# W298/Surtr

Hardware: AMD Instinct MI355X
Metric: fragments/sec (higher is better)
Workload: dtype f32

## Files before the change

surtr_amd/csrc/small_clip.h:

```cpp
#pragma once
#include "clip_core.h"

#define SC_V 192u
#define SC_H 640u
#define SC_FALLBACK 101

namespace surtr {

struct ScSolid
{
    float pos[3 * SC_V];
    uint32_t vw[SC_V];
    uint32_t re[SC_H];
};

struct ScLds
{
    ScSolid buf[2];
    int8_t c[SC_V];
    uint16_t km[SC_V];
    uint16_t mp[SC_V];
    uint16_t noff[SC_V];
    uint16_t succ[SC_V], pred[SC_V];
    uint32_t nv[2], flag;
#ifdef SURTR_STAMP
    unsigned long long tph[8];
#endif
};

__device__ inline int small_clip(const SolidIn in, const uint32_t F, const Shared& sh, ScLds& L, uint32_t* which, uint32_t* stop = nullptr)
{
    const uint32_t lane = lane_id();
    const uint32_t V = in.nv;
#ifdef SURTR_STAMP
    unsigned long long sc_t0 = __builtin_readcyclecounter();
    if (lane == 0) for (int q = 0; q < 8; ++q) L.tph[q] = 0;
#define SC_STAMP(i) do { if (lane == 0) { const unsigned long long t1 = __builtin_readcyclecounter(); L.tph[i] += t1 - sc_t0; sc_t0 = t1; } } while (0)
#else
#define SC_STAMP(i) do { } while (0)
#endif
    if (stop != nullptr) *stop = 0xFFFFFFFFu;
    if (V == 0 || V > SC_V) return SC_FALLBACK;
    const uint32_t hbase = in.loff[0], H = in.loff[V - 1u] + in.llen[V - 1u] - hbase;
    if (H > SC_H) return SC_FALLBACK;
    bool odd = false;
    for (uint32_t v = lane; v < V; v += SURTR_LANES)
    {
        ScSolid& S = L.buf[0];
        S.pos[3 * v] = in.pos[3 * v]; S.pos[3 * v + 1] = in.pos[3 * v + 1]; S.pos[3 * v + 2] = in.pos[3 * v + 2];
        const uint32_t lo = in.loff[v] - hbase, deg = in.llen[v];
        if (deg > 15u || deg < 3u) odd = true;
        const uint32_t dl = deg > 15u ? 15u : deg;
        S.vw[v] = lo | (dl << 16);
        const int32_t* r = in.nbr + in.loff[v];
        for (uint32_t j = 0; j < dl && lo + j < SC_H; ++j)
        {
            if ((uint32_t)r[j] >= V) odd = true;
            S.re[lo + j] = (uint32_t)r[j] & 0xFFFFu;
            for (uint32_t jj = 0; jj < j; ++jj) if (r[jj] == r[j]) odd = true;
        }
    }
    if (__ballot(odd) != 0ull) return SC_FALLBACK;
    __syncthreads();
    for (uint32_t v = lane; v < V; v += SURTR_LANES)
    {
        ScSolid& S = L.buf[0];
        const uint32_t w = S.vw[v], lo = w & 0xFFFFu, deg = w >> 16;
        for (uint32_t j = 0; j < deg; ++j)
        {
            const uint32_t e = S.re[lo + j] & 0xFFFFu;
            const uint32_t we = S.vw[e], elo = we & 0xFFFFu, edeg = we >> 16;
            uint32_t q = 0;
            while (q < edeg && (S.re[elo + q] & 0xFFFFu) != v) ++q;
            if (q >= edeg) odd = true;
            S.re[lo + j] = e | (q << 16);
        }
    }
    if (__ballot(odd) != 0ull) return SC_FALLBACK;
    __syncthreads();
    SC_STAMP(0);
#define SC_GIVE_UP do { if (stop != nullptr) { *stop = k; *which = cur; if (lane == 0) L.nv[cur] = nv; __syncthreads(); } return SC_FALLBACK; } while (0)
    uint32_t cur = 0, nv = V;
    for (uint32_t k = 0; k < F && nv != 0u; ++k)
    {
        const float4 pl = sh.planes[k];
        ScSolid& S = L.buf[cur]; ScSolid& N = L.buf[cur ^ 1u];
        bool zero = false, cut = false, keep = false;
        for (uint32_t v = lane; v < nv; v += SURTR_LANES)
        {
            const int c = side_of(plane_dist(pl, S.pos[3 * v], S.pos[3 * v + 1], S.pos[3 * v + 2]));
            L.c[v] = (int8_t)c;
            zero = zero || c == 0; cut = cut || c < 0; keep = keep || c > 0;
        }
        const bool anyCut = __ballot(cut) != 0ull;
        if (__ballot(keep) == 0ull) { if (!anyCut) SC_GIVE_UP; nv = 0; break; }
        if (!anyCut) continue;
        if (__ballot(zero) != 0ull) SC_GIVE_UP;
        __syncthreads();
        SC_STAMP(1);
        uint32_t carryM = 0, carryK = 0, carryH = 0;
        for (uint32_t v0 = 0; v0 < nv; v0 += SURTR_LANES)
        {
            const uint32_t v = v0 + lane;
            uint32_t mask = 0, isKept = 0, deg = 0;
            if (v < nv)
            {
                const uint32_t w = S.vw[v], lo = w & 0xFFFFu;
                deg = w >> 16;
                if (L.c[v] > 0) isKept = 1u;
                else
                    for (uint32_t j = 0; j < deg; ++j) if (L.c[S.re[lo + j] & 0xFFFFu] > 0) mask |= 1u << j;
            }
            const uint32_t cnt = (uint32_t)__builtin_popcount(mask);
            const uint2 inc = wave_incl_scan2(make_uint2(cnt | (isKept << 16), isKept ? deg : 0u));
            if (v < nv)
            {
                L.km[v] = (uint16_t)mask;
                L.mp[v] = isKept ? (uint16_t)(carryK + (inc.x >> 16) - 1u) : (uint16_t)(0x8000u | (carryM + (inc.x & 0xFFFFu) - cnt));
                L.noff[v] = (uint16_t)(carryH + inc.y - (isKept ? deg : 0u));
            }
            const uint32_t tx = lane_bcast(inc.x, SURTR_LANES - 1u), ty = lane_bcast(inc.y, SURTR_LANES - 1u);
            carryM += tx & 0xFFFFu; carryK += tx >> 16; carryH += ty;
        }
        const uint32_t M = carryM, nKeep = carryK, HK = carryH;
        if (nKeep + M > SC_V || HK + 3u * M > SC_H) SC_GIVE_UP;
        if (nKeep + M < 4u) { nv = 0; break; }
        for (uint32_t t = lane; t < M; t += SURTR_LANES) L.pred[t] = 0xFFFFu;
        __syncthreads();
        SC_STAMP(2);
        bool bad = false;
        for (uint32_t v = lane; v < nv; v += SURTR_LANES)
        {
            uint32_t mask = L.c[v] < 0 ? L.km[v] : 0u;
            if (!mask) continue;
            uint32_t t = L.mp[v] & 0x7FFFu;
            const uint32_t wv = S.vw[v];
            for (; mask; mask &= mask - 1u, ++t)
            {
                uint32_t cv = v, w = wv, slot = (uint32_t)__builtin_ctz(mask), steps = 0, end = 0xFFFFu;
                while (steps++ <= nv)
                {
                    const uint32_t len = w >> 16;
                    const uint32_t p = slot == 0u ? len - 1u : slot - 1u;
                    const uint32_t rw = S.re[(w & 0xFFFFu) + p];
                    const uint32_t e = rw & 0xFFFFu;
                    if (L.c[e] > 0) { end = (L.mp[cv] & 0x7FFFu) + (uint32_t)__builtin_popcount(L.km[cv] & ((1u << p) - 1u)); break; }
                    cv = e; slot = rw >> 16; w = S.vw[e];
                }
                if (end == 0xFFFFu || end == t) { bad = true; continue; }
                L.succ[t] = (uint16_t)end;
                L.pred[end] = (uint16_t)t;
            }
        }
        if (__ballot(bad) != 0ull) SC_GIVE_UP;
        __syncthreads();
        SC_STAMP(3);
        for (uint32_t t = lane; t < M; t += SURTR_LANES) if (L.pred[t] == 0xFFFFu || L.pred[L.succ[t]] != t || L.pred[t] == L.succ[t]) bad = true;
        if (__ballot(bad) != 0ull) SC_GIVE_UP;
        SC_STAMP(4);
        for (uint32_t v = lane; v < nv; v += SURTR_LANES)
        {
            const uint32_t w = S.vw[v], lo0 = w & 0xFFFFu, deg = w >> 16;
            if (L.c[v] > 0)
            {
                const uint32_t id = L.mp[v], lo = L.noff[v];
                N.pos[3 * id] = S.pos[3 * v]; N.pos[3 * id + 1] = S.pos[3 * v + 1]; N.pos[3 * id + 2] = S.pos[3 * v + 2];
                N.vw[id] = lo | (deg << 16);
                for (uint32_t j = 0; j < deg; ++j)
                {
                    const uint32_t rw = S.re[lo0 + j], e = rw & 0xFFFFu, q = rw >> 16;
                    const uint32_t m = L.mp[e], kme = L.km[e];
                    N.re[lo + j] = (m & 0x8000u) ? (nKeep + (m & 0x7FFFu) + (uint32_t)__builtin_popcount(kme & ((1u << q) - 1u))) | (2u << 16)
                                                 : m | (q << 16);
                }
            }
            else
            {
                const float ax = S.pos[3 * v], ay = S.pos[3 * v + 1], az = S.pos[3 * v + 2];
                const float sa = plane_dist(pl, ax, ay, az);
                uint32_t t = L.mp[v] & 0x7FFFu;
                for (uint32_t mask = L.km[v]; mask; mask &= mask - 1u, ++t)
                {
                    const uint32_t rw = S.re[lo0 + (uint32_t)__builtin_ctz(mask)], u = rw & 0xFFFFu;
                    const float bx = S.pos[3 * u], by = S.pos[3 * u + 1], bz = S.pos[3 * u + 2];
                    const float sb = plane_dist(pl, bx, by, bz);
                    const float inv = 1.f / (sb - sa);
                    const uint32_t id = nKeep + t, lo = HK + 3u * t;
                    N.pos[3 * id] = (ax * sb - bx * sa) * inv;
                    N.pos[3 * id + 1] = (ay * sb - by * sa) * inv;
                    N.pos[3 * id + 2] = (az * sb - bz * sa) * inv;
                    N.vw[id] = lo | (3u << 16);
                    N.re[lo] = (nKeep + L.pred[t]) | (1u << 16); N.re[lo + 1] = (nKeep + L.succ[t]) | (0u << 16);
                    N.re[lo + 2] = (uint32_t)L.mp[u] | (rw & 0xFFFF0000u);
                }
            }
        }
        nv = nKeep + M;
        cur ^= 1u;
        __syncthreads();
        SC_STAMP(5);
#ifdef SURTR_STAMP
        if (lane == 0) L.tph[6] += 1;
#endif
    }
#undef SC_GIVE_UP
    SC_STAMP(1);
    *which = cur;
    if (lane == 0) L.nv[cur] = nv;
    __syncthreads();
    return 0;
}

__device__ inline SolidIn sc_stage(const ScSolid& S, uint32_t nv, float* pos, uint32_t* loff, uint32_t* llen, uint32_t* ring)
{
    for (uint32_t v = lane_id(); v < nv; v += SURTR_LANES)
    {
        pos[3 * v] = S.pos[3 * v]; pos[3 * v + 1] = S.pos[3 * v + 1]; pos[3 * v + 2] = S.pos[3 * v + 2];
        const uint32_t w = S.vw[v], lo = w & 0xFFFFu, len = w >> 16;
        loff[v] = lo; llen[v] = len;
        for (uint32_t q = 0; q < len; ++q) ring[lo + q] = S.re[lo + q] & 0xFFFFu;
    }
    __threadfence_block();
    __syncthreads();
    return SolidIn{pos, loff, llen, (const int32_t*)ring, nv, nullptr, nullptr, nullptr, nullptr, nullptr};
}

__device__ inline int sc_park(const ScSolid& S, uint32_t nv, Shared& sh, uint32_t* cursors, float* apos, uint32_t* aloff, uint32_t* allen, int32_t* anbr,
                              uint32_t capV, uint32_t capH, uint32_t& voff, uint32_t& n, uint32_t& hoff, uint32_t& nh)
{
    const uint32_t wl = S.vw[nv - 1u];
    const uint32_t H = (wl & 0xFFFFu) + (wl >> 16);
    __syncthreads();
    if (threadIdx.x == 0) { sh.misc[0] = atomicAdd(&cursors[CUR_V], nv); sh.misc[1] = atomicAdd(&cursors[CUR_H], H); }
    __syncthreads();
    voff = sh.misc[0]; hoff = sh.misc[1];
    __syncthreads();
    if ((uint64_t)voff + nv > capV || (uint64_t)hoff + H > capH) return SURTR_E_CAPACITY;
    for (uint32_t v = lane_id(); v < nv; v += SURTR_LANES)
    {
        const size_t id = (size_t)voff + v;
        apos[3 * id] = S.pos[3 * v]; apos[3 * id + 1] = S.pos[3 * v + 1]; apos[3 * id + 2] = S.pos[3 * v + 2];
        const uint32_t w = S.vw[v];
        const uint32_t lo = hoff + (w & 0xFFFFu), len = w >> 16;
        aloff[id] = lo; allen[id] = len;
        const uint32_t* r = S.re + (w & 0xFFFFu);
        for (uint32_t q = 0; q < len; ++q) anbr[lo + q] = (int32_t)(r[q] & 0xFFFFu);
    }
    n = nv; nh = H;
    __syncthreads();
    return 0;
}

}
```

surtr_amd/csrc/surtr_ctx.h:

```cpp
#pragma once
#include <algorithm>
#include <chrono>
#include <cstdint>
#include <cstdlib>
#include <string>
#include <vector>

#include "../../include/surtr_hip.h"
#include "clip_core.h"

using namespace surtr;

struct PairRec
{
    uint32_t cv_off, cv_n, ch_off, ch_n;
    uint32_t mv_off, mv_n, mh_off, mh_n;
    uint32_t ni, isl_off;
    uint32_t status;
    uint32_t img_fmt, img_off, img_n, img_h, img_pc;
    uint32_t cv_bad;
};

enum { IMG_NONE = 0,
       IMG_NARROW = 1,
       IMG_WIDE = 2,
       IMG_EMPTY = 3,
       IMG_REC = 4 };

struct ImgLayout { uint32_t hist, zhist, nzero, mask, loff, llen, comp, ring, pos, total; };
__host__ __device__ static inline ImgLayout img_layout(uint32_t F, uint32_t nbV, uint32_t n, uint32_t hsum, uint32_t posCap = 0)
{
    auto up = [](uint32_t b) { return (b + 15u) & ~15u; };
    ImgLayout L;
    L.hist = 0; L.zhist = up(4u * F); L.nzero = L.zhist + up(4u * F); L.mask = L.nzero + up(4u * F); L.loff = L.mask + up(8u * nbV);
    L.llen = L.loff + up(2u * n); L.comp = L.llen + up(n); L.ring = L.comp + up(n); L.pos = L.ring + up(2u * hsum);
    L.total = L.pos + up(12u * (n > posCap ? n : posCap));
    return L;
}

struct ImgArena { char* base; uint32_t cap16; };

struct PrepPool { char* base; size_t per_wg; uint32_t VMAX; };
static size_t prep_bytes_per_wg(uint32_t VMAX)
{
    auto r = [](size_t b) { return (b + 255) & ~(size_t)255; };
    return 2 * r((size_t)VMAX * 4) + r((size_t)(VMAX / SURTR_SB + 2) * 4) + 2 * r((size_t)(VMAX / SURTR_LANES + 2) * 8) +
           2 * r((size_t)VMAX + 64) +
           2 * r((size_t)VMAX * 4) +
           r((size_t)VMAX * 2 + 64);
}

struct FragRec
{
    int32_t cell, piece, island;
    uint32_t mv_off, mv_n, mh_off, mh_n;
    uint32_t cv_off, cv_n, ch_off, ch_n;
    uint32_t idx_off, idx_n;
    uint32_t o_mv, o_mh, o_cv, o_ch, o_idx;
};

struct Arena
{
    float* pos; uint32_t* loff; uint32_t* llen; int32_t* nbr; uint32_t* idx;
    uint2* isl;
    uint32_t capV, capH, capI, capIsl;
    uint32_t* cursors;
};

enum : uint32_t
{
    CUR_V = 0,
    CUR_H = 1,
    CUR_I = 2,
    CUR_ISL = 3,
    CUR_Q_CLIP = 4,
    CUR_STATUS = 5,
    CUR_Q_REFIT = 6,
    CUR_Q_FACES = 7,
    CUR_Q_CONVEX = 8,
    CUR_Q_PREP = 9,
    CUR_IMG = 10,
    CUR_Q_BIG = 11,
    CUR_Q_HALF = 12,
    CUR_Q_RETRY = 13,
    CUR_FLAGGED_FRAGS = 14,
    CUR_FLAGGED_PAIRS = 15,
    CUR_CLS_CLIP = 16,
    CUR_CLS_FRAG = 32,
    CUR_CLS_PREP = 48,
    CUR_CLS_HALF = 64,
    CUR_RETRY_N = CUR_CLS_HALF,
    CUR_CVX_RESUMED = 78,
    CUR_REFIT_RESUMED = 79,
    CUR_CVX_TOOK = 80,
    CUR_REFIT_TOOK = 82,
    CUR_BIG_QUOTA = 84,
    CUR_FACES2_N = 85,
    CUR_Q_FACES2 = 86,
    CUR_REC_TOOK = 88,
    CUR_REC_HANDED = 89,
    CUR_LIT_TOO_LARGE = 90,
    CUR_REC_IMAGES = 91,
    CUR_SORTED_SEL = 92,
    CUR_REC_SPENT = 93,
    CUR_CATCH_CLIPPED = 94,
    CUR_UNREFITTED = 95,
    CUR_WC_WHY = 96,
    CUR_STATS_WORDS = 128,
    CUR_HO_PUSHED = 146,
    CUR_HO_STARTED = 147,
    CUR_HO_SIGNED_OFF = 148,
    CUR_HO_POLL_SLOT = 149,
    CUR_Q_CATCH = 150,
    CUR_Q_SWEEP = 151,
    CUR_HO_WORDS = 6,
    CUR_COUNT = 256
};
static_assert(CUR_V == 0 && CUR_H == 1 && CUR_I == 2 && CUR_ISL == 3 && CUR_STATUS == 5 && CUR_CLS_CLIP == 16 && CUR_CLS_FRAG == 32 &&
              CUR_CLS_PREP == 48 && CUR_CLS_HALF == 64 && CUR_REC_TOOK == 88 && CUR_REC_HANDED == 89 && CUR_LIT_TOO_LARGE == 90 &&
              CUR_UNREFITTED == 95 && CUR_WC_WHY == 96, "include/surtr_hip.h publishes these slots of surtr_queue_stats by number");
static_assert(CUR_STATS_WORDS <= CUR_COUNT && CUR_Q_SWEEP + 1 == CUR_HO_PUSHED + CUR_HO_WORDS && CUR_HO_PUSHED + CUR_HO_WORDS <= CUR_COUNT &&
              CUR_Q_FACES2 == CUR_FACES2_N + 1, "slot map");

struct alignas(16) SRow { uint32_t w[4]; };

struct Pieces
{
    const float* mpos; const uint32_t* mloff; const uint32_t* mllen; const int32_t* mnbr; const uint32_t* mvo; const uint8_t* mtri; const float* mrad;
    const uint32_t* mperm; const float4* mposr_s; const float4* mbsph; const uint32_t* mbo;
    const float* cpos; const uint32_t* cloff; const uint32_t* cllen; const int32_t* cnbr; const uint32_t* cvo; const uint8_t* ctri; const float* crad;
    const uint32_t* cperm; const float4* cposr_s; const float4* cbsph; const uint32_t* cbo;
    uint32_t n;
    const uint8_t* mdup; const uint8_t* cdup;
    const SRow* mrow_s; const uint32_t* miperm;
    const float4* mbsph2; const uint32_t* mbo2; const float4* mbsph3; const uint32_t* mbo3;
};

struct ScratchPool
{
    char* base; size_t per_wg;
    uint32_t CV, CH, VMAX;
};

struct Scratch
{
    float* pos;
    uint32_t* g_loff; uint32_t* g_llen; int8_t* g_comp; uint32_t* g_ring;
    uint32_t* g_succ; uint32_t* g_pred; uint32_t* g_pcnt;
    uint32_t* aux0; uint32_t* aux1; uint32_t* aux2; uint32_t* aux3;
    int8_t* g_gcomp;
    uint2* blk;
    unsigned long long* gmask; uint2* gblk;
    float* t_pos; uint32_t* t_loff; uint32_t* t_llen; int8_t* t_comp; uint32_t* t_ring;
    uint32_t CV, CH;
};

__device__ static Scratch carve(const ScratchPool& P, uint32_t wg)
{
    Scratch S;
    char* p = P.base + (size_t)wg * P.per_wg;
    auto take = [&](size_t bytes) { char* r = p; p += (bytes + 255) & ~(size_t)255; return r; };
    S.pos = (float*)take((size_t)P.CV * 12);
    S.g_loff = (uint32_t*)take((size_t)P.CV * 4);
    S.g_llen = (uint32_t*)take((size_t)P.CV * 4);
    S.g_comp = (int8_t*)take((size_t)P.CV);
    S.g_ring = (uint32_t*)take((size_t)P.CH * 4);
    S.g_succ = (uint32_t*)take((size_t)P.CV * 4);
    S.g_pred = (uint32_t*)take((size_t)P.CV * 4);
    S.g_pcnt = (uint32_t*)take((size_t)P.CV * 4);
    S.aux0 = (uint32_t*)take((size_t)P.CV * 4);
    S.aux1 = (uint32_t*)take((size_t)P.CV * 4);
    S.aux2 = (uint32_t*)take((size_t)P.CV * 4);
    S.aux3 = (uint32_t*)take((size_t)P.CV * 4);
    S.g_gcomp = (int8_t*)take((size_t)P.CV);
    S.blk = (uint2*)take((size_t)(P.CV / SURTR_LANES + 4) * 8);
    S.gmask = (unsigned long long*)take((size_t)(P.VMAX / SURTR_LANES + 2) * 8);
    S.gblk = (uint2*)take((size_t)(P.VMAX / SURTR_LANES + 2) * 8);
    S.t_pos = (float*)take((size_t)P.CV * 12); S.t_loff = (uint32_t*)take((size_t)P.CV * 4); S.t_llen = (uint32_t*)take((size_t)P.CV * 4);
    S.t_comp = (int8_t*)take((size_t)P.CV); S.t_ring = (uint32_t*)take((size_t)P.CH * 4);
    S.CV = P.CV; S.CH = P.CH;
    return S;
}

static size_t scratch_bytes_per_wg(uint32_t CV, uint32_t CH, uint32_t VMAX)
{
    auto r = [](size_t b) { return (b + 255) & ~(size_t)255; };
    return 2 * r((size_t)CV * 12) + 11 * r((size_t)CV * 4) + 3 * r((size_t)CV) + 2 * r((size_t)CH * 4) + r((size_t)(CV / SURTR_LANES + 4) * 8) +
           2 * r((size_t)(VMAX / SURTR_LANES + 2) * 8);
}

struct FaceScratch
{
    int32_t* base; size_t per_wg; uint32_t HF;
};

struct surtr_ctx;

template <class T>
struct DevBuf
{
    T* p = nullptr;
    size_t cap = 0;
    DevBuf() = default;
    DevBuf(DevBuf&& o) noexcept : p(o.p), cap(o.cap) { o.p = nullptr; o.cap = 0; }
    DevBuf& operator=(DevBuf&& o) noexcept { if (this != &o) { reset(); p = o.p; cap = o.cap; o.p = nullptr; o.cap = 0; } return *this; }
    ~DevBuf() { reset(); }
    void reset() { if (p) (void)hipFree(p); p = nullptr; cap = 0; }
    operator T*() const { return p; }
    int grow(surtr_ctx* ctx, size_t need, size_t alloc = 0);
};

struct PieceSet
{
    DevBuf<float> pos; DevBuf<uint32_t> loff, llen; DevBuf<int32_t> nbr; DevBuf<uint32_t> vo; DevBuf<uint8_t> tri; DevBuf<float> rad;
    DevBuf<uint32_t> perm; DevBuf<float4> posr_s, bsph; DevBuf<uint32_t> bo;
    DevBuf<float> box; DevBuf<unsigned long long> key, key2; DevBuf<uint32_t> val;
    DevBuf<uint8_t> dup;
    DevBuf<uint32_t> iperm; DevBuf<SRow> row_s;
    DevBuf<float4> bsph2; DevBuf<uint32_t> bo2; DevBuf<float4> bsph3; DevBuf<uint32_t> bo3;
};

struct CellBuffers
{
    DevBuf<double> seeds; DevBuf<uint32_t> goff; DevBuf<char> slots; DevBuf<uint32_t> cfo, cvo;
    DevBuf<int32_t> gen; DevBuf<uint32_t> fvo; DevBuf<double> verts; DevBuf<uint32_t> heads;
    uint32_t n = 0, nf = 0, nfv = 0;
};

#define SURTR_LVS (SURTR_LV / 2u)
#define SURTR_LHS ((SURTR_LH * 11u / 24u) & ~7u)
#ifndef SURTR_HALF_ROOM
#define SURTR_HALF_ROOM 2u
#endif
__host__ __device__ static inline bool fits_half(uint32_t n, uint32_t h, uint32_t capVs) { return SURTR_HALF_ROOM * n <= capVs && SURTR_HALF_ROOM * h <= SURTR_LHS; }
static inline bool surtr_fits_half(uint32_t n, uint32_t h) { return fits_half(n, h, SURTR_LVS); }

struct surtr_ctx
{
    int device = 0;
    bool frags_of_pieces = false;
    uint32_t hw_wg = 512, hw_wg_faces = 1024, hw_wg_prep = 1792, hw_wg_big = 48, budget_vmax = 0xFFFFFFFFu, budget_hmax = 0xFFFFFFFFu;
    uint32_t max_wg = 512, max_wg_faces = 1024, max_wg_small = 2048, max_wg_prep = 1792, max_wg_half = 1024;
    DevBuf<uint32_t> d_hlist;
    uint32_t vmin = 0;
    ScratchPool pool_half{}; uint32_t n_wg_half = 0; DevBuf<char> pool_half_buf;
    bool half_on = false;
    PrepPool prep{nullptr, 0, 0}; uint32_t n_wg_prep = 0; DevBuf<char> prep_buf;
    ImgArena img{nullptr, 0}; DevBuf<char> img_buf;
    DevBuf<uint32_t> d_order;
    DevBuf<uint32_t> d_forder;
    bool wave_big = false;
    uint32_t n_wg_big = 48;
    hipStream_t stream2 = nullptr;
    hipStream_t stream3 = nullptr;
    hipEvent_t ev_prep = nullptr, ev_big = nullptr, ev_half = nullptr, ev_cvx = nullptr;
    uint32_t events_in_flight = 1;
    hipStream_t stream = nullptr;
    std::string err;
    uint32_t n_pieces = 0, vmax = 0, hmax = 0, cvmax = 0, chmax = 0;
    CellBuffers cells;
    PieceSet mset, cset;
    DevBuf<uint32_t> d_upload_err;
    DevBuf<float> d_group_xf;
    DevBuf<float> d_world;
    DevBuf<char> sort_tmp;
    DevBuf<uint32_t> d_from;
    DevBuf<uint32_t> d_qstatus; uint32_t qstatus_n = 0;
    float upload_ms = 0.f; uint32_t upload_allocs = 0;
    std::vector<uint32_t> scene_off;
    std::vector<uint32_t> h_vo[2], h_ho[2];
    int scene_event_compound = -1;
    std::vector<float> scene_pose;
    bool scene_dev_stale = true;
    std::vector<double> h_pose_stage; std::vector<uint32_t> h_comp_stage;
    DevBuf<double> d_pose;
    DevBuf<uint32_t> d_piece_comp;
    struct { DevBuf<float> pos; DevBuf<uint32_t> loff; DevBuf<int32_t> nbr; DevBuf<uint32_t> vo; } spare[2];
    DevBuf<int32_t> d_commit_src; DevBuf<uint32_t> d_commit_tab;
    float commit_ms[2] = {0.f, 0.f};
    uint32_t regroup_rounds = 0;
    uint64_t tot_mv = 0, tot_mh = 0;
    uint32_t n_cells = 0, n_faces = 0;
    DevBuf<uint32_t> d_pair_order; uint32_t pair_order_begin = 0, pair_order_count = 0;
    bool pair_order_is_list = false;
    DevBuf<float> d_v012; DevBuf<float4> d_planes; DevBuf<uint32_t> d_plane_off;
    std::vector<uint32_t> h_plane_off;
    bool planes_ready = false;
    uint32_t user_cv = 0, user_ch = 0;
    uint64_t user_av = 0, user_ah = 0, user_ai = 0;
    ScratchPool pool{}; uint32_t n_wg = 0; DevBuf<char> pool_buf;
    ScratchPool pool_small{}; uint32_t n_wg_small = 0; DevBuf<char> pool_small_buf;
    FaceScratch fs{}; DevBuf<int32_t> fs_buf; DevBuf<uint2> d_blk; uint32_t blk_per_wg = 0, n_wg_faces_alloc = 0;
    FaceScratch fs_big{}; DevBuf<int32_t> fs_big_buf; DevBuf<uint2> d_blk_big; uint32_t blk_per_wg_big = 0, n_wg_faces_big = 0;
    DevBuf<uint32_t> d_face_list;
    Arena arena{};
    struct { DevBuf<float> pos; DevBuf<uint32_t> loff, llen, idx, cursors; DevBuf<int32_t> nbr; DevBuf<uint2> isl; } arena_buf;
    DevBuf<PairRec> d_pairs;
    DevBuf<FragRec> d_frags; uint32_t cap_frags = 0;
    DevBuf<uint32_t> d_frag_status;
    DevBuf<uint2> d_scanblk;
    DevBuf<surtr_counts> d_counts;
    DevBuf<uint32_t> d_face_group;
    DevBuf<uint8_t> d_outside;
    std::vector<uint8_t> last_outside;
    DevBuf<uint2> d_pair_list;
    uint32_t refit_limit = 4;
    DevBuf<uint32_t> d_hull_ws;
    float color[3] = {0.25f, 0.25f, 0.25f};
    surtr_counts last{}; bool last_current = false;
    bool have_event = false; uint32_t last_flags = 0;
    DevBuf<char> d_blob;
    bool profiling = false;
    hipEvent_t hev[16][2] = {}; uint32_t hcount = 0; int hslot[16] = {};
    hipEvent_t ev[32] = {};
    bool ev_valid[16] = {};
};

#define PROF_BEGIN_ON(i, strm) do { if (ctx->profiling) { (void)hipEventRecord(ctx->ev[2 * (i)], strm); } } while (0)
#define PROF_END_ON(i, strm) do { if (ctx->profiling) { (void)hipEventRecord(ctx->ev[2 * (i) + 1], strm); ctx->ev_valid[i] = true; } } while (0)
#define PROF_HIST_BEGIN(i, strm) do { if (ctx->profiling && ctx->hev[0][0]) { (void)hipEventRecord(ctx->hev[ctx->hcount % 16u][0], strm); } } while (0)
#define PROF_HIST_END(i, strm) do { if (ctx->profiling && ctx->hev[0][0]) { (void)hipEventRecord(ctx->hev[ctx->hcount % 16u][1], strm); ctx->hslot[ctx->hcount % 16u] = (i); ++ctx->hcount; } } while (0)
#define PROF_BEGIN(i) PROF_BEGIN_ON(i, st)
#define PROF_END(i) PROF_END_ON(i, st)

#define HIPCHK(call)                                                                              \
    do {                                                                                          \
        hipError_t e_ = (call);                                                                   \
        if (e_ != hipSuccess) { ctx->err = std::string(#call) + ": " + hipGetErrorString(e_); return SURTR_E_HIP; } \
    } while (0)

template <class T>
int DevBuf<T>::grow(surtr_ctx* ctx, size_t need, size_t alloc)
{
    if (p && cap >= need) return SURTR_OK;
    reset();
    const size_t n = std::max(need, alloc);
    const hipError_t e = hipMalloc((void**)&p, n * sizeof(T));
    if (e != hipSuccess)
    {
        p = nullptr;
        (void)hipGetLastError();
        ctx->err = "device allocation of " + std::to_string(n * sizeof(T)) + " bytes: " + hipGetErrorString(e);
        return SURTR_E_HIP;
    }
    cap = n;
    return SURTR_OK;
}

namespace pieces {
template <class T>
int grow_pieces(surtr_ctx* ctx, DevBuf<T>& b, size_t need)
{
    const size_t cap0 = b.cap;
    const int rc = b.grow(ctx, need, std::max<size_t>(need + need / 4, 64));
    if (rc == SURTR_OK && b.cap != cap0) ++ctx->upload_allocs;
    return rc;
}
struct Timer
{
    surtr_ctx* ctx; std::chrono::steady_clock::time_point t0;
    explicit Timer(surtr_ctx* c) : ctx(c), t0(std::chrono::steady_clock::now()) { c->upload_allocs = 0; }
    ~Timer() { ctx->upload_ms = std::chrono::duration<float, std::milli>(std::chrono::steady_clock::now() - t0).count(); }
};
int reserve_set(surtr_ctx* ctx, PieceSet& S, uint32_t n, uint32_t V, uint32_t H, uint32_t NB);
int derive_set(surtr_ctx* ctx, PieceSet& S, uint32_t n, uint32_t V, const std::vector<uint32_t>& bo_h, bool check, uint32_t H = 0xFFFFFFFFu);
std::vector<uint32_t> sphere_offsets(uint32_t n, const uint32_t* vo);
void set_piece_stats(surtr_ctx* ctx, uint32_t n, const uint32_t* mvo, const uint32_t* mho, const uint32_t* cvo, const uint32_t* cho);
int finish_upload(surtr_ctx* ctx, uint32_t n, bool check);
int transform_range(surtr_ctx* ctx, uint32_t p0, uint32_t n, const float* world);
}
struct SceneDev { const double* pose; const uint32_t* piece_comp; const uint32_t* comp_off; uint32_t n_comp; };
static inline void scene_reset_poses(surtr_ctx* ctx) { ctx->scene_pose.clear(); ctx->scene_dev_stale = true; }
static inline int scene_sync_device(surtr_ctx* ctx, SceneDev* out)
{
    if (ctx->scene_off.size() < 2 || ctx->scene_off.back() != ctx->n_pieces) return SURTR_E_STATE;
    const uint32_t nc = (uint32_t)ctx->scene_off.size() - 1u, np = ctx->n_pieces;
    if (ctx->scene_dev_stale || !ctx->d_pose || !ctx->d_piece_comp)
    {
        std::vector<double>& P = ctx->h_pose_stage; std::vector<uint32_t>& C = ctx->h_comp_stage;
        P.assign((size_t)12 * nc, 0.0); C.resize((size_t)np + nc + 1u);
        for (uint32_t c = 0; c < nc; ++c)
        {
            double* m = P.data() + (size_t)12 * c;
            if (ctx->scene_pose.empty()) { m[0] = m[4] = m[8] = 1.0; }
            else
            {
                const float* W = ctx->scene_pose.data() + (size_t)16 * c;
                for (int r = 0; r < 3; ++r) { for (int k = 0; k < 3; ++k) m[3 * r + k] = (double)W[4 * k + r]; m[9 + r] = (double)W[4 * r + 3]; }
            }
            for (uint32_t p = ctx->scene_off[c]; p < ctx->scene_off[c + 1]; ++p) C[p] = c;
        }
        for (uint32_t c = 0; c <= nc; ++c) C[(size_t)np + c] = ctx->scene_off[c];
        int rc = ctx->d_pose.grow(ctx, P.size(), P.size() + P.size() / 4);
        if (rc == SURTR_OK) rc = ctx->d_piece_comp.grow(ctx, C.size(), C.size() + C.size() / 4);
        if (rc) return rc;
        HIPCHK(hipMemcpyAsync(ctx->d_pose.p, P.data(), P.size() * 8, hipMemcpyHostToDevice, ctx->stream));
        HIPCHK(hipMemcpyAsync(ctx->d_piece_comp.p, C.data(), C.size() * 4, hipMemcpyHostToDevice, ctx->stream));
        ctx->scene_dev_stale = false;
    }
    *out = SceneDev{ctx->d_pose.p, ctx->d_piece_comp.p, ctx->d_piece_comp.p + np, nc};
    return SURTR_OK;
}

int surtr_event_pairs_masked(surtr_ctx* ctx, uint32_t n_pairs, const uint32_t* pair_cell, const uint32_t* pair_piece, const uint8_t* outside, uint32_t flags);
int surtr_event_regroup_skipped(surtr_ctx* ctx, const std::vector<uint32_t>& skipped, int partial, uint32_t n_sphere, const float* sphere_points,
                                const float origin[3], float radius, uint32_t* n_pieces, uint32_t* n_compounds, uint32_t* compound_off, int32_t* compound_piece);

extern "C" int surtr_place_cells_groups_dev(surtr_ctx* ctx, uint32_t n_groups, const uint32_t* group_cell_off, const float* d_scale3, const float* d_shift3);
```

surtr_amd/csrc/surtr_hip.hip:

```cpp
#include <algorithm>
#include <cmath>
#include <cstdio>
#include <cstdlib>
#include <cstring>
#include <string>
#include <type_traits>
#include <vector>

#include "surtr_ctx.h"
#include "small_clip.h"
#ifndef SC_RESUME
#define SC_RESUME 1
#endif
#include "literal_clip.h"
#include "wave_clip.h"
#include "prep_sorted.h"

template <uint32_t LV, uint32_t LH>
struct alignas(16) LdsTopoT
{
    static_assert(LV % 16 == 0 && LH % 8 == 0, "clip_image copies 16-byte words into these arrays");
    static constexpr uint32_t kLV = LV, kLH = LH;
    alignas(16) uint16_t loff[LV];
    alignas(16) uint8_t llen[LV];
// ... 346 lines not shown
                    uint2 c = make_uint2(0u, 0u);
                    if (i < nA) c = lenfn(i);
                    const uint2 e = wave_excl2(c);
                    if (i < nA) roff[i] = (uint16_t)(T.blk[b].x + e.x);
                }
                uint32_t voff, hoff, ioff;
                if (!arena_take(A, sh, nA, hh, 1u, voff, hoff, ioff)) return SURTR_E_CAPACITY;
                for (uint32_t i = tid; i < nA; i += group_size())
                {
                    const uint32_t v = alist[i], id = voff + i;
                    A.pos[3 * (size_t)id] = T.pos[3 * v]; A.pos[3 * (size_t)id + 1] = T.pos[3 * v + 1]; A.pos[3 * (size_t)id + 2] = T.pos[3 * v + 2];
                    const uint32_t lo = hoff + roff[i], len = T.llen[v];
                    A.loff[id] = lo; A.llen[id] = len;
                    const I* r = T.ring + T.loff[v];
                    for (uint32_t q = 0; q < len; ++q) A.nbr[lo + q] = (int32_t)pidx[(uint32_t)r[q]];
                }
                if (tid == 0) A.isl[ioff] = make_uint2(nA, hh);
                rec.mv_off = voff; rec.mv_n = nA; rec.mh_off = hoff; rec.mh_n = hh; rec.ni = 1u; rec.isl_off = ioff;
                __syncthreads();
                STAMP(83);
                return 0;
            }
        }
    }
    const uint2 tot = index_live(T, sh);
    STAMP(80);
    uint32_t* lab = T.aux1;
    for (uint32_t v = tid; v < nS; v += group_size()) lab[v] = v;
    __syncthreads();
    while (true)
    {
        if (tid == 0) sh.changed = 0;
        __syncthreads();
        bool ch = false;
        for (uint32_t v = tid; v < nS; v += group_size())
        {
            if (!T.alive(v)) continue;
            uint32_t m = lab[v];
            const I* r = T.ring + T.loff[v];
            const uint32_t len = T.llen[v];
            for (uint32_t q = 0; q < len; ++q) { const uint32_t o = lab[(uint32_t)r[q]]; m = o < m ? o : m; }
            const uint32_t mm = lab[m];
            m = mm < m ? mm : m;
            if (m < lab[v]) { lab[v] = m; ch = true; }
        }
        if (ch) sh.changed = 1;
        __syncthreads();
        const bool more = sh.changed != 0;
        __syncthreads();
        if (!more) break;
    }
    STAMP(81);
    auto rootfn = [&](uint32_t v) -> uint2 { return make_uint2((T.alive(v) && lab[v] == v) ? 1u : 0u, 0u); };
    uint32_t ni = 0, dum = 0;
    scan_blocks(nS, T.blk, sh, rootfn, ni, dum);
    uint32_t voff, hoff, ioff;
    if (!arena_take(A, sh, tot.x, tot.y, ni, voff, hoff, ioff)) return SURTR_E_CAPACITY;
    STAMP(82);
    if (ni == 1)
    {
        write_solid(T, A.pos, A.loff, A.llen, A.nbr, voff, hoff);
        if (tid == 0) A.isl[ioff] = tot;
    }
    else
    {
        uint32_t* irank = T.aux2; uint32_t* local = T.aux0;
        const uint32_t nb = (nS + SURTR_LANES - 1u) >> SURTR_LSH;
        for (uint32_t b = wave_id(); b < nb; b += group_waves())
        {
            const uint32_t v = (b << SURTR_LSH) + lane_id();
            uint2 c = make_uint2(0u, 0u);
            if (v < nS) c = rootfn(v);
            const uint2 e = wave_excl2(c);
            if (v < nS && c.x) irank[v] = T.blk[b].x + e.x;
        }
        __syncthreads();
        uint32_t vbase = 0, hbase = 0;
        for (uint32_t t = 0; t < ni; ++t)
        {
            auto isfn = [&](uint32_t v) -> uint2 {
                return (T.alive(v) && irank[lab[v]] == t) ? make_uint2(1u, (uint32_t)T.llen[v]) : make_uint2(0u, 0u);
            };
            uint32_t tv = 0, th = 0;
            scan_blocks(nS, T.blk, sh, isfn, tv, th);
            for (uint32_t b = wave_id(); b < nb; b += group_waves())
            {
                const uint32_t v = (b << SURTR_LSH) + lane_id();
                uint2 c = make_uint2(0u, 0u);
                if (v < nS) c = isfn(v);
                const uint2 e = wave_excl2(c);
                if (v < nS && c.x)
                {
                    const uint32_t lv = T.blk[b].x + e.x;
                    const uint32_t dv = voff + vbase + lv;
                    local[v] = lv;
                    A.pos[3 * (size_t)dv] = T.pos[3 * v]; A.pos[3 * (size_t)dv + 1] = T.pos[3 * v + 1];
                    A.pos[3 * (size_t)dv + 2] = T.pos[3 * v + 2];
                    A.llen[dv] = c.y;
                    A.loff[dv] = hoff + hbase + T.blk[b].y + e.y;
                }
            }
            if (tid == 0) A.isl[ioff + t] = make_uint2(tv, th);
            __syncthreads();
            for (uint32_t v = tid; v < nS; v += group_size())
            {
                if (!T.alive(v) || irank[lab[v]] != t) continue;
                const uint32_t dv = voff + vbase + local[v];
                const I* r = T.ring + T.loff[v];
                int32_t* d = A.nbr + A.loff[dv];
                const uint32_t len = T.llen[v];
                for (uint32_t q = 0; q < len; ++q) d[q] = (int32_t)local[(uint32_t)r[q]];
            }
            vbase += tv; hbase += th;
            __syncthreads();
        }
    }
    rec.mv_off = voff; rec.mv_n = tot.x; rec.mh_off = hoff; rec.mh_n = tot.y; rec.ni = ni; rec.isl_off = ioff;
    __syncthreads();
    STAMP(83);
    return 0;
}

__device__ __attribute__((noinline)) static ParkOut solid_global(SolidIn in, uint32_t F, ScratchPool pool, uint32_t wg, Arena A, Shared* shp)
{
    Shared& sh = *shp;
    Scratch S = carve(pool, wg);
    ParkOut o{0, 0u, 0u, 0u, 0u, false};
    o.err = clip_global(in, F, S, sh, [&](auto& T) -> int {
        if (T.nLive == 0) return 0;
        return park_topo(T, sh, A, o.voff, o.n, o.hoff, o.nh);
    });
    return o;
}

__device__ __forceinline__ static bool solid_is_sliver_inl(const SolidIn& in)
{
    bool odd = false;
    for (uint32_t v = threadIdx.x; v < in.nv; v += group_size())
    {
        const int32_t* r = in.nbr + in.loff[v];
        const uint32_t deg = in.llen[v];
        for (uint32_t j = 0; j < deg; ++j)
        {
            const int32_t u = r[j];
            for (uint32_t q = 0; q < j; ++q) if (r[q] == u) odd = true;
            if (u < 0 || (uint32_t)u >= in.nv) { odd = true; continue; }
            const int32_t* ru = in.nbr + in.loff[u];
            const uint32_t du = in.llen[u];
            bool back = false;
            for (uint32_t q = 0; q < du; ++q) if (ru[q] == (int32_t)v) back = true;
            if (!back) odd = true;
        }
    }
    return __syncthreads_or(odd ? 1 : 0) != 0;
}
__device__ static bool solid_is_sliver(const SolidIn in) { return solid_is_sliver_inl(in); }

struct LitRun { int err; uint32_t n, nh; LitSolid LS; const uint32_t* off; bool stale; };
__device__ __attribute__((noinline)) static LitRun literal_run(SolidIn in, uint32_t F, ScratchPool pool, uint32_t wg, Shared* shp, bool ids_set = false,
                                                                uint32_t* too_big = nullptr)
{
    Shared& sh = *shp;
    Scratch S = carve(pool, wg);
    const uint32_t capV = S.CV < S.CH / LIT_STRIDE ? S.CV : S.CH / LIT_STRIDE;
    LitRun r{SURTR_E_TOPOLOGY, 0u, 0u, LitSolid{S.pos, S.g_loff, (int32_t*)S.g_ring, S.g_llen, (int32_t*)S.t_ring, S.g_comp, (int32_t*)S.aux0, capV}, S.aux1, false};
    __syncthreads();
    if (threadIdx.x == 0)
    {
        uint32_t n = 0; bool stale = false;
        int rc = literal_clip(in, F, sh.planes, r.LS, &n, &stale, ids_set);
        if (rc == SURTR_E_CAPACITY) { rc = SURTR_E_TOPOLOGY; if (too_big != nullptr) atomicAdd(too_big, 1u); }
        uint32_t h = 0;
        if (rc == 0) for (uint32_t v = 0; v < n; ++v) { S.aux1[v] = h; h += r.LS.len[v]; }
        sh.misc[2] = (uint32_t)rc; sh.misc[3] = n; sh.misc[4] = h; sh.misc[5] = stale ? 1u : 0u;
    }
    __syncthreads();
    r.err = (int)sh.misc[2]; r.n = sh.misc[3]; r.nh = sh.misc[4]; r.stale = sh.misc[5] != 0u;
    __syncthreads();
    return r;
}
__device__ static void literal_write(const LitRun& r, float* pos, uint32_t* loff, uint32_t* llen, int32_t* nbr, uint32_t voff, uint32_t hoff)
{
    for (uint32_t v = threadIdx.x; v < r.n; v += group_size())
    {
        const size_t id = (size_t)voff + v;
        pos[3 * id] = r.LS.pos[3 * v]; pos[3 * id + 1] = r.LS.pos[3 * v + 1]; pos[3 * id + 2] = r.LS.pos[3 * v + 2];
        const uint32_t lo = hoff + r.off[v], len = r.LS.len[v];
        loff[id] = lo; llen[id] = len;
        for (uint32_t q = 0; q < len; ++q) nbr[lo + q] = r.LS.ring[v * LIT_STRIDE + q];
    }
    __syncthreads();
}
__device__ __attribute__((noinline)) static ParkOut solid_literal(SolidIn in, uint32_t F, ScratchPool pool, uint32_t wg, Arena A, Shared* shp, bool ids_set = false)
{
    const LitRun r = literal_run(in, F, pool, wg, shp, ids_set, &A.cursors[CUR_LIT_TOO_LARGE]);
    ParkOut o{r.err, 0u, 0u, 0u, 0u, r.stale};
    if (r.err != 0 || r.n == 0u) return o;
    uint32_t ioff;
    if (!arena_take(A, *shp, r.n, r.nh, 0, o.voff, o.hoff, ioff)) { o.err = SURTR_E_CAPACITY; return o; }
    literal_write(r, A.pos, A.loff, A.llen, A.nbr, o.voff, o.hoff);
    o.n = r.n; o.nh = r.nh;
    return o;
}

struct ChainCaller
{
    uint32_t slot_took, slot_resumed;
    bool count_literal_first;
    float4* keep;
    const float4* restore_from;
};
struct LiteralArg { SolidIn in; bool ids_set; };
struct ChainStamp { unsigned long long t_small, t_park; int path; };
template <class Literal>
__device__ __forceinline__ ParkOut convex_chain(const SolidIn cin, const uint32_t F, bool literal_first, const ChainCaller who, Literal&& literal,
                                                Shared& sh, OneWaveLds& U, Scratch& S, const ScratchPool& pool, const Arena& A, ChainStamp& st)
{
    const uint32_t tid = threadIdx.x;
    ParkOut o{SURTR_E_TOPOLOGY, 0u, 0u, 0u, 0u, false};
    uint32_t which = 0, stop = 0xFFFFFFFFu;
#ifdef SURTR_NO_SMALL_CLIP
    literal_first = false;
    o.err = SC_FALLBACK;
#else
    if (!literal_first) o.err = small_clip(cin, F, sh, U.f, &which, &stop);
#endif
    if (tid == 0 && (!literal_first || who.count_literal_first)) atomicAdd(&A.cursors[who.slot_took + (o.err == 0 ? 0u : 1u)], 1u);
#ifdef SURTR_STAMP
    st.t_small = st.t_park = __builtin_readcyclecounter();
#endif
    if (!literal_first)
    {
        if (o.err == 0)
        {
            const uint32_t nv = U.f.nv[which];
            if (nv != 0u) o.err = sc_park(U.f.buf[which], nv, sh, A.cursors, A.pos, A.loff, A.llen, A.nbr, A.capV, A.capH, o.voff, o.n, o.hoff, o.nh);
        }
        __syncthreads();
#ifdef SURTR_STAMP
        st.t_park = __builtin_readcyclecounter();
#endif
        if (o.err == SC_FALLBACK)
        {
            SolidIn cx = cin; uint32_t Fx = F;
            const bool resumed = SC_RESUME && stop != 0xFFFFFFFFu && stop > 0u && stop < F;
            if (resumed)
            {
                const uint32_t nvs = U.f.nv[which];
                cx = sc_stage(U.f.buf[which], nvs, S.pos, S.g_loff, S.g_llen, S.g_ring);
                Fx = F - stop;
                for (uint32_t k = tid; k < F; k += group_size())
                {
                    const float4 pk = sh.planes[k];
                    if (who.keep != nullptr) who.keep[k] = pk;
                    sh.pmar[k] = pk;
                }
                __syncthreads();
                for (uint32_t k = tid; k < Fx; k += group_size()) sh.planes[k] = sh.pmar[k + stop];
                __syncthreads();
                if (tid == 0) atomicAdd(&A.cursors[who.slot_resumed], 1u);
            }
            o.err = clip_any<false>(cx, Fx, S, sh, U.g.L, [&](auto& T) -> int {
                if (T.nLive == 0) return 0;
                return park_topo(T, sh, A, o.voff, o.n, o.hoff, o.nh);
            }, &U.g.W);
            __syncthreads();
            if (resumed)
            {
                for (uint32_t k = tid; k < F; k += group_size()) sh.planes[k] = who.restore_from[k];
                __syncthreads();
            }
        }
#ifdef SURTR_STAMP
        if (o.err == SURTR_OVERFLOW) st.path |= 1;
        if (o.err == SURTR_E_TOPOLOGY) st.path |= 2;
#endif
        if (o.err == SURTR_OVERFLOW)
        {
            o = solid_global(cin, F, pool, blockIdx.x, A, &sh);
            __syncthreads();
        }
    }
    if (o.err == SURTR_E_TOPOLOGY)
    {
#ifdef SURTR_STAMP
        st.path |= 4;
#endif
        const LiteralArg la = literal();
        const ParkOut l = solid_literal(la.in, F, pool, blockIdx.x, A, &sh, la.ids_set);
        if (l.err == 0) o = l;
        else if (l.err != SURTR_E_TOPOLOGY) o.err = l.err;
        __syncthreads();
    }
    return o;
}

#ifndef SURTR_LITERAL_MESH_V
#define SURTR_LITERAL_MESH_V 2048u
#define SURTR_LITERAL_START_V 64u
#endif
#ifndef SURTR_SMALL_WAVES
#define SURTR_SMALL_WAVES 2
#endif
__global__ __launch_bounds__(SURTR_LANES) __attribute__((amdgpu_waves_per_eu(SURTR_SMALL_WAVES, 8))) void k_clip_convex(Pieces P, const float4* __restrict__ planes,
                                                    const uint32_t* __restrict__ plane_off, uint32_t cell_begin,
                                                    uint32_t n_pairs, const uint8_t* __restrict__ outside,
                                                    ScratchPool pool, Arena A, PairRec* __restrict__ pairs,
                                                    const uint2* __restrict__ pair_list, uint32_t* __restrict__ porder,
                                                    const uint32_t* __restrict__ pair_order, uint32_t front_par)
{
    __shared__ Shared sh;
    __shared__ OneWaveLds U;
    LdsTopoSmall& L = U.g.L; LdsWorkSmall& W = U.g.W;
    Scratch S = carve(pool, blockIdx.x);
    const uint32_t tid = threadIdx.x;
    while (true)
    {
        __syncthreads();
        if (tid == 0) sh.misc[7] = atomicAdd(&A.cursors[CUR_Q_CONVEX], 1u);
        __syncthreads();
        uint32_t p = sh.misc[7];
        if (p >= n_pairs) break;
        if (pair_order != nullptr) p = pair_order[p];
        const PairAt at = pair_where(p, pair_list, cell_begin, P.n);
        const uint32_t cell = at.cell, piece = at.piece;
        PairRec rec;
        memset(&rec, 0, sizeof(rec));
#ifdef SURTR_STAMP_SMALL
        if (tid == 0) for (int q = 0; q < 16; ++q) sh.ph[q] = 0;
#endif
        bool skip = outside != nullptr && outside[piece] != 0;
        const uint32_t f0 = plane_off[cell], F = plane_off[cell + 1] - f0;
        if (F > SURTR_MAXF) { rec.status = SURTR_E_INVALID; skip = true; }
        int err = 0;
        ChainStamp cst{};
#ifdef SURTR_STAMP
        const unsigned long long cx0 = __builtin_readcyclecounter();
        cst.t_small = cst.t_park = cx0;
#endif
        if (!skip)
        {
            for (uint32_t k = tid; k < F; k += group_size()) sh.planes[k] = planes[f0 + k];
            __syncthreads();
            const ChainCaller who{CUR_CVX_TOOK, CUR_CVX_RESUMED, true, nullptr, planes + f0};
            const ParkOut o = convex_chain(convex_solid_in(P, piece), F, P.cdup[piece] != 0, who, [&] { return LiteralArg{convex_solid_in(P, piece), false}; }, sh, U, S, pool, A, cst);
            err = o.err; rec.cv_off = o.voff; rec.cv_n = o.n; rec.ch_off = o.hoff; rec.ch_n = o.nh;
        }
        if (err == SURTR_E_TOPOLOGY) { rec.cv_bad = 1; rec.cv_off = 0; rec.cv_n = 1; rec.ch_off = 0; rec.ch_n = 0; err = 0; }
        if (err != 0) { rec.status = (uint32_t)err; rec.cv_n = 0; if (tid == 0) atomicMax(&A.cursors[CUR_STATUS], (uint32_t)err); }
        if (tid == 0)
        {
            if (!front_par) pairs[p] = rec;
            else
            {
                PairRec& o = pairs[p];
                o.cv_off = rec.cv_off; o.cv_n = rec.cv_n; o.ch_off = rec.ch_off; o.ch_n = rec.ch_n;
                o.mv_off = 0; o.mv_n = 0; o.mh_off = 0; o.mh_n = 0; o.ni = 0; o.isl_off = 0; o.status = rec.status; o.cv_bad = rec.cv_bad;
            }
        }
        if (rec.cv_n != 0 && porder != nullptr)
        {
            const uint32_t m0 = P.mvo[piece], V = P.mvo[piece + 1] - m0;
            const float4* bs = P.mbsph + P.mbo[piece];
            const uint32_t nsb = (V + SURTR_SB - 1u) / SURTR_SB;
            __syncthreads();
            for (uint32_t k = tid; k < F; k += group_size())
            {
                const float4 pk = sh.planes[k];
                const float n1 = fabsf(pk.x) + fabsf(pk.y) + fabsf(pk.z);
                const float n2 = sqrtf(pk.x * pk.x + pk.y * pk.y + pk.z * pk.z) * 1.0001f;
                sh.pmar[k] = make_float4(n2 * 1.00101f, 1.0e-5f * fabsf(pk.w), 1.0e-5f * n1, 0.f);
            }
            __syncthreads();
            uint32_t und = 0;
            for (uint32_t sb = tid * 8u; sb < nsb; sb += group_size() * 8u)
            {
                const float4 sp = bs[sb];
                const float mag = fabsf(sp.x) + fabsf(sp.y) + fabsf(sp.z) + sp.w;
                bool decided = false;
                for (uint32_t k = 0; k < F; ++k)
                {
                    const float4 mk = sh.pmar[k];
                    const float sk = plane_dist(sh.planes[k], sp.x, sp.y, sp.z);
                    const float margin = sp.w * mk.x + mk.y + mk.z * mag;
                    if (sk > margin) { decided = true; break; }
                    if (!(sk < -margin)) break;
                }
                if (!decided) ++und;
            }
            const uint2 tot = wave_incl_scan2(make_uint2(und, 0u));
            if (tid == group_size() - 1u)
            {
                uint32_t l2 = 0; while ((tot.x >> (l2 + 1u)) != 0u) ++l2;
                uint32_t cls = 2u * l2 + (l2 ? ((tot.x >> (l2 - 1u)) & 1u) : 0u);
                cls = cls > 4u ? cls - 4u : 0u; if (cls > 15u) cls = 15u;
                porder[(size_t)cls * n_pairs + atomicAdd(&A.cursors[CUR_CLS_PREP + cls], 1u)] = p;
            }
        }
#ifdef SURTR_STAMP_SMALL
        if (tid == 0) for (int q = 0; q < 16; ++q) if (sh.ph[q]) atomicAdd(&g_stamp[q], sh.ph[q]);
#endif
#ifdef SURTR_STAMP
        if (tid == 0)
        {
            const unsigned long long cx1 = cst.t_small, cx2 = cst.t_park, cx3 = __builtin_readcyclecounter();
            const unsigned long long d = cx3 - cx0;
            atomicAdd(&g_stamp2[32], d); atomicAdd(&g_stamp2[33], 1ull);
            const unsigned long long old = atomicMax(&g_stamp2[34], d);
            if (d > old)
            {
                g_stamp2[35] = cx1 - cx0; g_stamp2[36] = cx2 - cx1; g_stamp2[37] = cx3 - cx2; g_stamp2[38] = F;
                for (int q = 0; q < 7; ++q) g_stamp2[40 + q] = U.f.tph[q];
            }
        }
#endif
    }
}

#ifndef SURTR_PREP_MINV
#define SURTR_PREP_MINV 2048u
#endif
#ifndef SURTR_PREP_NB
#define SURTR_PREP_NB 1024u
#endif
#ifndef SURTR_PREP_WAVES
#define SURTR_PREP_WAVES 7
#endif
template <bool OLD_SELECT = true>
__device__ __attribute__((always_inline)) static inline void prep_pairs_body(Shared& sh, unsigned long long* lmask, uint2* lblk, uint32_t rec_on,
                                                         const Pieces& P, const float4* __restrict__ planes,
                                                         const uint32_t* __restrict__ plane_off, uint32_t cell_begin,
                                                         uint32_t n_pairs, const PrepPool& pool, const Arena& A, const ImgArena& IA, uint32_t capV, uint32_t capVs,
                                                         PairRec* __restrict__ pairs, const uint2* __restrict__ pair_list,
                                                         uint32_t* __restrict__ order, const uint32_t* __restrict__ porder,
                                                         uint32_t* __restrict__ horder, uint32_t half_on, uint32_t big_quota, uint32_t big_n)
{
    auto enqueue = [&](uint32_t p, uint32_t cls) { order[(size_t)cls * n_pairs + atomicAdd(&A.cursors[CUR_CLS_CLIP + cls], 1u)] = p; };
    auto enqueue_half = [&](uint32_t p, uint32_t cls) { horder[(size_t)cls * n_pairs + atomicAdd(&A.cursors[CUR_CLS_HALF + cls], 1u)] = p; };
    const uint32_t tid = threadIdx.x;
    const bool front_par = (rec_on & 4u) != 0u;
    char* sp = pool.base + (size_t)blockIdx.x * pool.per_wg;
    auto take = [&](size_t bytes) { char* r = sp; sp += (bytes + 255) & ~(size_t)255; return r; };
    uint32_t* needy = (uint32_t*)take((size_t)pool.VMAX * 4);
    uint32_t* orig = (uint32_t*)take((size_t)pool.VMAX * 4);
    uint32_t* und = (uint32_t*)take((size_t)(pool.VMAX / SURTR_SB + 2) * 4);
    unsigned long long* gmask = (unsigned long long*)take((size_t)(pool.VMAX / SURTR_LANES + 2) * 8);
    uint2* gblk = (uint2*)take((size_t)(pool.VMAX / SURTR_LANES + 2) * 8);
    uint8_t* vfc = (uint8_t*)take((size_t)pool.VMAX + 64);
    uint8_t* fcb = (uint8_t*)take((size_t)pool.VMAX + 64);
    uint32_t* klist = (uint32_t*)take((size_t)pool.VMAX * 4);
    uint32_t* walks = (uint32_t*)take((size_t)pool.VMAX * 4);
    uint16_t* sid16 = (uint16_t*)take((size_t)pool.VMAX * 2 + 64);
#ifdef SURTR_STAMP
    const unsigned long long wg_t0 = __builtin_readcyclecounter();
    unsigned long long wg_work = 0;
#endif
    while (true)
    {
        __syncthreads();
        if (tid == 0)
        {
            uint32_t t = atomicAdd(&A.cursors[CUR_Q_PREP], 1u);
            if (front_par) sh.misc[7] = t < n_pairs ? t : 0xFFFFFFFFu;
            else sh.misc[7] = pair_of_ticket(A, porder, n_pairs, t, CUR_CLS_PREP, 15, 0);
        }
        __syncthreads();
        const uint32_t p = sh.misc[7];
        if (p >= n_pairs) break;
        const PairAt at = pair_where(p, pair_list, cell_begin, P.n);
        const uint32_t cell = at.cell, piece = at.piece;
        if (front_par)
        {
            if (tid == 0) { pairs[p].img_fmt = IMG_NONE; pairs[p].img_off = 0; pairs[p].img_n = 0; pairs[p].img_h = 0; pairs[p].img_pc = 0; }
            if (plane_off[cell + 1] - plane_off[cell] > SURTR_MAXF) continue;
        }
        else if (pairs[p].cv_n == 0 || pairs[p].status != 0) continue;
        const uint32_t m0 = P.mvo[piece], V = P.mvo[piece + 1] - m0;
        if (V < SURTR_PREP_MINV || V > pool.VMAX)
        {
            if (tid == 0)
            {
                const bool sliver = P.mdup[piece] != 0 && V <= SURTR_LITERAL_START_V;
                if (half_on && !sliver && V <= pool.VMAX && fits_half(V, P.mloff[m0 + V] - P.mloff[m0], capVs)) enqueue_half(p, 1u);
                else enqueue(p, V > pool.VMAX ? 13u : 0u);
            }
            continue;
        }
#ifdef SURTR_STAMP
        const unsigned long long pair_t0 = __builtin_readcyclecounter();
#endif
        STAMP_DECL;
        const uint32_t f0 = plane_off[cell], F = plane_off[cell + 1] - f0;
        for (uint32_t k = tid; k < F; k += group_size()) sh.planes[k] = planes[f0 + k];
        __syncthreads();
        SolidIn min{P.mpos + 3 * (size_t)m0, P.mloff + m0, P.mllen + m0, P.mnbr, V, P.mtri + m0, P.mrad + m0,
                    P.mperm + m0, P.mposr_s + m0, P.mbsph + P.mbo[piece]};
        STAMP(70);
        const uint32_t nbV = (V + SURTR_LANES - 1u) >> SURTR_LSH;
        unsigned long long* bmask = nbV <= SURTR_PREP_NB ? lmask : gmask;
        uint2* bblk = nbV <= SURTR_PREP_NB ? lblk : gblk;
        uint32_t n = 0, hsum = 0;
#ifndef SURTR_PREP_G
#define SURTR_PREP_G 1
#define SURTR_PREP_NBATCH 4
#endif
        constexpr uint32_t kUbWords = (SURTR_PREP_NB - SURTR_PS_NB) * 2u;
        const bool sorted_sel = !(rec_on & 2u) && nbV <= SURTR_PREP_NB && (V + SURTR_SB - 1u) / SURTR_SB <= 32u * kUbWords && V < 0xFFFFu && P.mrow_s != nullptr;
        if (sorted_sel)
        {
            const SortedRings sr{P.mrow_s + m0, P.miperm + m0, P.mbsph2 + P.mbo2[piece], P.mbsph3 + P.mbo3[piece]};
            prepass_select_sorted<SURTR_PREP_NB, kUbWords>(min, sr, F, sh, (unsigned char*)lmask, vfc, (uint16_t*)needy, (uint16_t*)und, klist, walks, n, hsum);
        }
        else if constexpr (OLD_SELECT) prepass_select<SURTR_PREP_G, SURTR_PREP_NBATCH>(min, F, sh, bmask, bblk, needy, und, n, hsum);
        const bool toolong = sh.flagBad != 0;
        __syncthreads();
        STAMP(71);
        uint32_t fmt = IMG_NARROW, off16 = 0;
        if (!OLD_SELECT && !sorted_sel) fmt = IMG_NONE;
        else if (n == 0) fmt = IMG_EMPTY;
        else if (toolong || n > 2u * capV || hsum > 2u * SURTR_LH || n >= InLds::SENT) fmt = IMG_WIDE;
        const bool to_half = half_on && fits_half(n, hsum, capVs);
        const bool rec_fmt = (rec_on & 1u) != 0u && sorted_sel && fmt == IMG_NARROW && !to_half && F <= WC_MAXF && n < WC_MAXN && n <= (rec_on >> 8) &&
                             sh.misc[5] == 0u && sh.deg7 == 0u && P.mdup[piece] == 0 &&
                             (fits_with_room(n, hsum, capV, SURTR_LH) || big_quota == 0xFFFFFFFFu);
        uint32_t ncut_rec = 0, maxb_rec = 0;
        if (rec_fmt)
        {
            const RecLayout rl = rec_layout(F, n);
            const uint32_t need16 = rl.total / 16u;
            if (tid == 0) sh.misc[0] = atomicAdd(&A.cursors[CUR_IMG], need16);
            __syncthreads();
            off16 = sh.misc[0];
            __syncthreads();
            if ((uint64_t)off16 + need16 > IA.cap16) fmt = IMG_NONE;
            else
            {
                prepass_emit_records(min, F, sh, bmask, bblk, klist, orig, fcb, sid16, sh.pw, IA.base + (size_t)off16 * 16u, n, ncut_rec, maxb_rec);
                fmt = IMG_REC;
            }
        }
        const uint32_t posCap = to_half ? 0u : (fits_with_room(n, hsum, capV, SURTR_LH) ? capV : 2u * capV);
        const ImgLayout lay = img_layout(F, nbV, n, hsum, posCap);
        if (fmt == IMG_NARROW && !rec_fmt)
        {
            const uint32_t need16 = lay.total / 16u;
            if (tid == 0) sh.misc[0] = atomicAdd(&A.cursors[CUR_IMG], need16);
            __syncthreads();
            off16 = sh.misc[0];
            __syncthreads();
            if ((uint64_t)off16 + need16 > IA.cap16) fmt = IMG_NONE;
        }
        STAMP(72);
        if (fmt == IMG_NARROW)
        {
            char* img = IA.base + (size_t)off16 * 16u;
            unsigned long long* gm = (unsigned long long*)(img + lay.mask);
            for (uint32_t b = tid; b < nbV; b += group_size()) gm[b] = bmask[b];
            STAMP(73);
            Topo<InLds> T;
            T.loff = (uint16_t*)(img + lay.loff); T.llen = (uint8_t*)(img + lay.llen); T.fc = (uint8_t*)(img + lay.comp); T.gcomp = nullptr;
            T.ring = (uint16_t*)(img + lay.ring); T.pos = (float*)(img + lay.pos);
            T.succ = T.pred = T.pcnt = T.aux0 = T.aux1 = T.aux2 = T.aux3 = nullptr; T.blk = nullptr;
            T.capV = n; T.capH = hsum; T.nS = T.nLive = T.hUsed = 0; T.kcur = T.n0cur = 0; T.zmode = false;
            if (tid < 4u) sh.cutmask[tid] = 0u;
            __syncthreads();
            if (sorted_sel) prepass_emit_klist(min, F, sh, T, bmask, bblk, klist, orig, (uint2*)und, n, hsum, maxb_rec);
            else if constexpr (OLD_SELECT) prepass_emit(min, F, sh, T, bmask, bblk, orig, n, hsum);
            STAMP(74);
            prepass_finish_hist(F, sh);
            uint32_t* hs = (uint32_t*)(img + lay.hist); uint32_t* zs = (uint32_t*)(img + lay.zhist); uint32_t* nz = (uint32_t*)(img + lay.nzero);
            for (uint32_t k = tid; k < F; k += group_size()) { hs[k] = sh.hist[k]; zs[k] = sh.zhist[k]; nz[k] = sh.nzero[k]; }
            STAMP(75);
        }
        if (tid == 0)
        {
            pairs[p].img_fmt = fmt; pairs[p].img_off = off16; pairs[p].img_n = n; pairs[p].img_h = hsum; pairs[p].img_pc = posCap;
            if (fmt == IMG_REC) atomicAdd(&A.cursors[CUR_REC_IMAGES], 1u);
            if (sorted_sel) atomicAdd(&A.cursors[CUR_SORTED_SEL], 1u);
            uint32_t cls = 15u;
            if (fmt == IMG_NONE) cls = 13u;
            else if (fmt == IMG_NARROW || fmt == IMG_REC)
            {
                const uint32_t ncut = fmt == IMG_REC ? ncut_rec : (uint32_t)(__builtin_popcount(sh.cutmask[0]) + __builtin_popcount(sh.cutmask[1]) +
                                                 __builtin_popcount(sh.cutmask[2]) + __builtin_popcount(sh.cutmask[3]));
                const uint32_t cost = (41u * ncut + n / 40u) / 110u;
                cls = !fits_with_room(n, hsum, capV, SURTR_LH) ? 14u : 1u + (cost < 11u ? cost : 11u);
                if (cls < 12u && fmt == IMG_NARROW) { bool inplane = false; for (uint32_t k = 0; k < F; ++k) if (sh.nzero[k] != 0u) inplane = true; if (inplane) cls = 12u; }
            }
            if (big_quota == 0xFFFFFFFFu)
            {
                if (cls >= 14u && !((fmt == IMG_NARROW || fmt == IMG_REC) && n < WC_MAXN)) cls = 13u;
                else if (cls < 12u && (fmt == IMG_NARROW || fmt == IMG_REC) && n > big_n && n < WC_MAXN) cls = 14u;
            }
            else if (cls >= 14u && fmt != IMG_EMPTY && atomicAdd(&A.cursors[CUR_BIG_QUOTA], 1u) >= big_quota) cls = 13u;
            if (fmt == IMG_NARROW && to_half) enqueue_half(p, cls < 6u ? cls : 6u);
            else if (fmt != IMG_EMPTY) enqueue(p, cls);
        }
#ifdef SURTR_STAMP
        if (tid == 0) { const unsigned long long d = __builtin_readcyclecounter() - pair_t0; wg_work += d; int bkt = 0; while ((d >> bkt) > 1 && bkt < 30) ++bkt; bkt = bkt < 16 ? 0 : bkt - 16; if (bkt > 7) bkt = 7; atomicAdd(&g_stamp[62 + bkt], 1ull); }
#endif
    }
#ifdef SURTR_STAMP
    if (tid == 0) { const unsigned long long d = __builtin_readcyclecounter() - wg_t0; atomicAdd(&g_stamp[56], d); atomicMax(&g_stamp[57], d); atomicAdd(&g_stamp[58], 1ull); atomicAdd(&g_stamp[59], wg_work); atomicMax(&g_stamp[60], wg_work); }
#endif
}

__global__ __launch_bounds__(SURTR_WG) __attribute__((amdgpu_waves_per_eu(SURTR_PREP_WAVES, 8))) void k_prep_pairs(Pieces P, const float4* __restrict__ planes,
                                                         const uint32_t* __restrict__ plane_off, uint32_t cell_begin,
                                                         uint32_t n_pairs, PrepPool pool, Arena A, ImgArena IA, uint32_t capV, uint32_t capVs,
                                                         PairRec* __restrict__ pairs, const uint2* __restrict__ pair_list,
                                                         uint32_t* __restrict__ order, const uint32_t* __restrict__ porder,
                                                         uint32_t* __restrict__ horder, uint32_t half_on, uint32_t big_quota, uint32_t big_n, uint32_t rec_on)
{
    __shared__ Shared sh;
    __shared__ unsigned long long lbuf[2u * SURTR_PREP_NB];
    unsigned long long* lmask = lbuf; uint2* lblk = (uint2*)(lbuf + SURTR_PREP_NB);
    prep_pairs_body(sh, lmask, lblk, rec_on, P, planes, plane_off, cell_begin, n_pairs, pool, A, IA, capV, capVs, pairs, pair_list, order, porder, horder, half_on, big_quota, big_n);
}

__global__ __launch_bounds__(SURTR_WG) __attribute__((amdgpu_waves_per_eu(SURTR_PREP_WAVES, 8))) void k_prep_pairs_sorted(Pieces P, const float4* __restrict__ planes,
                                                         const uint32_t* __restrict__ plane_off, uint32_t cell_begin,
                                                         uint32_t n_pairs, PrepPool pool, Arena A, ImgArena IA, uint32_t capV, uint32_t capVs,
                                                         PairRec* __restrict__ pairs, const uint2* __restrict__ pair_list,
                                                         uint32_t* __restrict__ order, const uint32_t* __restrict__ porder,
                                                         uint32_t* __restrict__ horder, uint32_t half_on, uint32_t big_quota, uint32_t big_n, uint32_t rec_on)
{
    __shared__ Shared sh;
    __shared__ unsigned long long lbuf[2u * SURTR_PREP_NB];
    unsigned long long* lmask = lbuf; uint2* lblk = (uint2*)(lbuf + SURTR_PREP_NB);
    prep_pairs_body<false>(sh, lmask, lblk, rec_on, P, planes, plane_off, cell_begin, n_pairs, pool, A, IA, capV, capVs, pairs, pair_list, order, porder, horder, half_on, big_quota, big_n);
}

__global__ __launch_bounds__(SURTR_WG_WIDE) void k_prep_pairs_wide(Pieces P, const float4* __restrict__ planes,
                                                         const uint32_t* __restrict__ plane_off, uint32_t cell_begin,
                                                         uint32_t n_pairs, PrepPool pool, Arena A, ImgArena IA, uint32_t capV, uint32_t capVs,
                                                         PairRec* __restrict__ pairs, const uint2* __restrict__ pair_list,
                                                         uint32_t* __restrict__ order, const uint32_t* __restrict__ porder,
                                                         uint32_t* __restrict__ horder, uint32_t half_on, uint32_t big_quota, uint32_t big_n, uint32_t rec_on)
{
    __shared__ Shared sh;
    __shared__ unsigned long long lbuf[2u * SURTR_PREP_NB];
    unsigned long long* lmask = lbuf; uint2* lblk = (uint2*)(lbuf + SURTR_PREP_NB);
    prep_pairs_body(sh, lmask, lblk, rec_on, P, planes, plane_off, cell_begin, n_pairs, pool, A, IA, capV, capVs, pairs, pair_list, order, porder, horder, half_on, big_quota, big_n);
}

__device__ __attribute__((noinline)) static int pair_global(Pieces P, uint32_t piece, uint32_t F, ScratchPool pool, uint32_t wg, Arena A,
                                                            Shared* shp, PairRec* pairs, uint32_t p, uint32_t literal)
{
    Shared& sh = *shp;
    Scratch S = carve(pool, wg);
    PairRec rec = pairs[p];
    SolidIn min = mesh_solid_in(P, piece);
    auto consume = [&](auto& T) -> int {
        if (T.nLive == 0) return 0;
        return park_mesh_islands(T, sh, A, rec);
    };
    int err = 0;
    bool gone = false;
    if (literal != 0u)
    {
        const ParkOut o = solid_literal(min, F, pool, wg, A, shp);
        err = o.err;
        gone = err == 0 && o.n == 0u;
        if (err == 0 && o.n != 0u)
        {
            min = SolidIn{A.pos + 3 * (size_t)o.voff, A.loff + o.voff, A.llen + o.voff, A.nbr, o.n, nullptr, nullptr, nullptr, nullptr, nullptr};
            F = 0u;
        }
        __syncthreads();
    }
    if (err == 0 && !gone) err = clip_global(min, F, S, sh, consume);
    __syncthreads();
    return finish_pair(A, pairs, p, rec, err);
}

template <bool HALF = false, class LT>
__device__ __attribute__((always_inline)) static inline void clip_pair_general(Shared& sh, LT& L, Scratch& S, const ScratchPool& pool, uint32_t wg, const Pieces& P,
                                       const float4* __restrict__ planes, const uint32_t* __restrict__ plane_off, uint32_t cell_begin,
                                       const Arena& A, const ImgArena& IA, PairRec* __restrict__ pairs, const uint2* __restrict__ pair_list,
                                       uint32_t* __restrict__ horder, const uint32_t p, PairRec rec)
{
    const uint32_t tid = threadIdx.x;
    const PairAt at = pair_where(p, pair_list, cell_begin, P.n);
    const uint32_t cell = at.cell, piece = at.piece;
    const uint32_t f0 = plane_off[cell], F = plane_off[cell + 1] - f0;
    for (uint32_t k = tid; k < F; k += group_size()) sh.planes[k] = planes[f0 + k];
    __syncthreads();
    SolidIn min = mesh_solid_in(P, piece);
    auto consume = [&](auto& T) -> int {
        if (T.nLive == 0) return 0;
        return park_mesh_islands(T, sh, A, rec);
    };
    if (P.mdup[piece] != 0 && min.nv <= SURTR_LITERAL_START_V)
    {
        if (HALF) { if (tid == 0) horder[atomicAdd(&A.cursors[CUR_RETRY_N], 1u)] = p; }
        else pair_global(P, piece, F, pool, wg, A, &sh, pairs, p, 1u);
        return;
    }
    int err;
    if (HALF)
    {
        if (rec.img_fmt == IMG_NARROW) err = clip_image<false>(IA.base + (size_t)rec.img_off * 16u, rec.img_n, rec.img_h, 0u, min, F, S, sh, L, consume);
        else err = clip_any<false>(min, F, S, sh, L, consume);
        __syncthreads();
        if (err == SURTR_OVERFLOW)
        {
            if (tid == 0) horder[atomicAdd(&A.cursors[CUR_RETRY_N], 1u)] = p;
            return;
        }
    }
    else
    {
        err = SURTR_OVERFLOW;
        if (rec.img_fmt == IMG_NARROW) err = clip_image<false>(IA.base + (size_t)rec.img_off * 16u, rec.img_n, rec.img_h, rec.img_pc, min, F, S, sh, L, consume);
        else if (rec.img_fmt != IMG_WIDE) err = clip_any<false>(min, F, S, sh, L, consume);
        __syncthreads();
        if (err == SURTR_OVERFLOW)
        {
// ... 1474 lines not shown
        }
#if SURTR_LANES == 64
        for (uint32_t f0 = 0; f0 < (fan ? 0u : nfaces); f0 += SURTR_LANES)
        {
            const uint32_t fl = f0 + lane_id();
            uint32_t mylo = 0, mylen = 0;
            if (fl < nfaces) { mylo = (uint32_t)faceLo[fl]; mylen = (uint32_t)faceLen[fl]; }
            unsigned long long todo = __ballot(mylen >= 5u && mylen <= SURTR_EAR_WAVE_MAX);
            for (uint32_t ord = 0; todo != 0ull; todo &= todo - 1ull, ++ord)
            {
                if (ord % group_waves() != wave_id()) continue;
                const uint32_t src = (uint32_t)__builtin_ctzll(todo);
                const uint32_t lo = lane_bcast(mylo, src), len = lane_bcast(mylen, src);
                uint32_t cnt;
                if (len > 64u) cnt = ear_clip_face_wave_k<SURTR_EAR_WAVE_MAX / 64>(pos, (const int32_t*)loopbuf + lo, (int)len, tri + 3u * (size_t)lo);
                else if (ear_lds) cnt = ear_clip_face_wave((const float*)FU.ear.pos, (const uint16_t*)FU.ear.loop + lo, (int)len, tri + 3u * (size_t)lo);
                else cnt = ear_clip_face_wave(pos, (const int32_t*)loopbuf + lo, (int)len, tri + 3u * (size_t)lo);
                if (lane_id() == 0) fcnt[f0 + src] = cnt;
            }
        }
        __syncthreads();
        STAMP(63);
#endif
        for (uint32_t fi = tid; fi < (fan ? 0u : nfaces); fi += group_size())
        {
            const uint32_t lo = (uint32_t)faceLo[fi], len = (uint32_t)faceLen[fi];
#if SURTR_LANES == 64
            if (len >= 5u && len <= SURTR_EAR_WAVE_MAX) continue;
#endif
            uint32_t* out = tri + 3u * (size_t)lo;
            uint32_t cnt = 0u;
            if (len >= 3u && len <= 8u)
                cnt = ear_lds ? ear_clip_small((const float*)FU.ear.pos, (const uint16_t*)FU.ear.loop + lo, (int)len, out)
                              : ear_clip_small(pos, (const int32_t*)loopbuf + lo, (int)len, out);
            else if (len > 8u) cnt = ear_clip_face(pos, (const int32_t*)loopbuf + lo, (int)len, eartmp + 3 * (size_t)lo, out);
            fcnt[fi] = cnt;
#ifdef SURTR_STAMP
            if (len > 64u) { atomicAdd(&g_stamp[66], 1ull); atomicAdd(&g_stamp[67], (unsigned long long)len); }
#endif
        }
        __syncthreads();
        STAMP(64);
        auto cntfn = [&](uint32_t fi) -> uint2 { return make_uint2(fcnt[fi], 0u); };
        uint32_t nidx = 0, dum = 0;
        scan_blocks(nfaces, blk, sh, cntfn, nidx, dum);
        if (tid == 0) sh.misc[0] = atomicAdd(&A.cursors[CUR_I], nidx);
        __syncthreads();
        const uint32_t ioff = sh.misc[0];
        if ((uint64_t)ioff + nidx > A.capI) { if (tid == 0) atomicMax(&A.cursors[CUR_STATUS], (uint32_t)SURTR_E_CAPACITY); continue; }
        {
            const uint32_t nb = (nfaces + SURTR_LANES - 1u) >> SURTR_LSH;
            for (uint32_t b = wave_id(); b < nb; b += group_waves())
            {
                const uint32_t fi = (b << SURTR_LSH) + lane_id();
                uint2 c = make_uint2(0u, 0u);
                if (fi < nfaces) c = cntfn(fi);
                const uint2 ex = wave_excl2(c);
                if (fi < nfaces && c.x)
                {
                    const uint32_t* src = tri + 3u * (size_t)(uint32_t)faceLo[fi];
                    uint32_t* dst = A.idx + ioff + blk[b].x + ex.x;
                    for (uint32_t q = 0; q < c.x; ++q) dst[q] = src[q];
                }
            }
        }
        if (tid == 0) { frags[f].idx_off = ioff; frags[f].idx_n = nidx; }
        STAMP(65);
#ifdef SURTR_STAMP
        if (tid == 0)
        {
            const unsigned long long d = __builtin_readcyclecounter() - frag_t0;
            int bkt = 0; while ((d >> bkt) > 1 && bkt < 40) ++bkt; bkt = bkt < 12 ? 0 : bkt - 12; if (bkt > 15) bkt = 15;
            atomicAdd(&g_stamp2[32 + bkt], 1ull); atomicAdd(&g_stamp2[51], d);
            for (int q = 0; q < 6; ++q) atomicAdd(&g_stamp2[24 + q], sh.ph[(60 + q) & 15]);
            const unsigned long long old = atomicMax(&g_stamp2[48], d);
            if (d > old) { g_stamp2[49] = n; g_stamp2[50] = H; g_stamp2[55] = nfaces; for (int q = 0; q < 6; ++q) g_stamp2[56 + q] = sh.ph[(60 + q) & 15]; }
        }
#endif
    }
#ifdef SURTR_STAMP
    if (tid == 0) { const unsigned long long d = __builtin_readcyclecounter() - wg_t0f; atomicAdd(&g_stamp2[52], d); atomicMax(&g_stamp2[53], d); atomicAdd(&g_stamp2[54], 1ull); }
#endif
}

__global__ __launch_bounds__(SURTR_WG_WIDE) void k_out_scan(FragRec* __restrict__ frags, uint2* __restrict__ blk,
                                                       surtr_counts* __restrict__ counts, Arena A)
{
    __shared__ Shared sh;
    const uint32_t nf = counts->n_frag;
    const uint32_t nb = (nf + SURTR_LANES - 1u) >> SURTR_LSH;
    uint32_t t0 = 0, t1 = 0;
    auto f1 = [&](uint32_t f) -> uint2 { return make_uint2(frags[f].mv_n, frags[f].mh_n); };
    scan_blocks(nf, blk, sh, f1, t0, t1);
    for (uint32_t b = wave_id(); b < nb; b += group_waves())
    {
        const uint32_t f = (b << SURTR_LSH) + lane_id();
        uint2 c = make_uint2(0u, 0u);
        if (f < nf) c = f1(f);
        const uint2 e = wave_excl2(c);
        if (f < nf) { frags[f].o_mv = blk[b].x + e.x; frags[f].o_mh = blk[b].y + e.y; }
    }
    const uint32_t mv = t0, mh = t1;
    __syncthreads();
    auto f2 = [&](uint32_t f) -> uint2 { return make_uint2(frags[f].cv_n, frags[f].ch_n); };
    scan_blocks(nf, blk, sh, f2, t0, t1);
    for (uint32_t b = wave_id(); b < nb; b += group_waves())
    {
        const uint32_t f = (b << SURTR_LSH) + lane_id();
        uint2 c = make_uint2(0u, 0u);
        if (f < nf) c = f2(f);
        const uint2 e = wave_excl2(c);
        if (f < nf) { frags[f].o_cv = blk[b].x + e.x; frags[f].o_ch = blk[b].y + e.y; }
    }
    const uint32_t cv = t0, chh = t1;
    __syncthreads();
    auto f3 = [&](uint32_t f) -> uint2 { return make_uint2(frags[f].idx_n, 0u); };
    scan_blocks(nf, blk, sh, f3, t0, t1);
    for (uint32_t b = wave_id(); b < nb; b += group_waves())
    {
        const uint32_t f = (b << SURTR_LSH) + lane_id();
        uint2 c = make_uint2(0u, 0u);
        if (f < nf) c = f3(f);
        const uint2 e = wave_excl2(c);
        if (f < nf) frags[f].o_idx = blk[b].x + e.x;
    }
    if (threadIdx.x == 0)
    {
        counts->mesh_verts = mv; counts->mesh_nbrs = mh; counts->conv_verts = cv; counts->conv_nbrs = chh;
        counts->n_idx = t0; counts->status = A.cursors[CUR_STATUS]; counts->n_failed = A.cursors[CUR_FLAGGED_FRAGS] + A.cursors[CUR_FLAGGED_PAIRS];
    }
}

struct BlobLayout
{
    size_t ids, mvo, mpos, mno, mnbr, cvo, cpos, cno, cnbr, vnc, ioff, idx, fstat, total;
};

__host__ __device__ static BlobLayout blob_layout(const surtr_counts& c)
{
    BlobLayout L;
    size_t at = 64;
    auto put = [&](size_t bytes) { size_t r = at; at += (bytes + 63) & ~(size_t)63; return r; };
    L.ids = put((size_t)c.n_frag * 12);
    L.mvo = put(((size_t)c.n_frag + 1) * 4);
    L.mpos = put((size_t)c.mesh_verts * 12);
    L.mno = put(((size_t)c.mesh_verts + 1) * 4);
    L.mnbr = put((size_t)c.mesh_nbrs * 4);
    L.cvo = put(((size_t)c.n_frag + 1) * 4);
    L.cpos = put((size_t)c.conv_verts * 12);
    L.cno = put(((size_t)c.conv_verts + 1) * 4);
    L.cnbr = put((size_t)c.conv_nbrs * 4);
    L.vnc = put((size_t)c.mesh_verts * 36);
    L.ioff = put(((size_t)c.n_frag + 1) * 4);
    L.idx = put((size_t)c.n_idx * 4);
    L.fstat = put((size_t)c.n_frag * 4);
    L.total = at;
    return L;
}

__global__ __launch_bounds__(SURTR_WG) void k_pack(const FragRec* __restrict__ frags, surtr_counts* __restrict__ counts,
                                                   Arena A, char* __restrict__ blob, size_t capacity, uint32_t with_vnc,
                                                   const uint32_t* __restrict__ frag_status, float cr, float cg, float cb)
{
    const surtr_counts c = *counts;
    const BlobLayout L = blob_layout(c);
    if (L.total > capacity)
    {
        if (blockIdx.x == 0 && threadIdx.x == 0)
        {
            atomicMax(&A.cursors[CUR_STATUS], (uint32_t)SURTR_E_CAPACITY);
            atomicMax(&counts->status, (uint32_t)SURTR_E_CAPACITY);
            if (capacity >= sizeof(surtr_counts))
            {
                surtr_counts z; memset(&z, 0, sizeof(z)); z.n_pairs = c.n_pairs; z.status = SURTR_E_CAPACITY;
                *(surtr_counts*)blob = z;
            }
        }
        return;
    }
    const uint32_t nf = c.n_frag, tid = threadIdx.x;
    if (blockIdx.x == 0 && tid == 0)
    {
        *(surtr_counts*)blob = c;
        ((uint32_t*)(blob + L.mvo))[nf] = c.mesh_verts;
        ((uint32_t*)(blob + L.mno))[c.mesh_verts] = c.mesh_nbrs;
        ((uint32_t*)(blob + L.cvo))[nf] = c.conv_verts;
        ((uint32_t*)(blob + L.cno))[c.conv_verts] = c.conv_nbrs;
        ((uint32_t*)(blob + L.ioff))[nf] = c.n_idx;
    }
    for (uint32_t f = blockIdx.x; f < nf; f += gridDim.x)
    {
        const FragRec fr = frags[f];
        if (tid == 0)
        {
            int32_t* ids = (int32_t*)(blob + L.ids);
            ids[3 * f] = fr.cell; ids[3 * f + 1] = fr.piece; ids[3 * f + 2] = fr.island;
            ((uint32_t*)(blob + L.mvo))[f] = fr.o_mv;
            ((uint32_t*)(blob + L.cvo))[f] = fr.o_cv;
            ((uint32_t*)(blob + L.ioff))[f] = fr.o_idx;
            ((uint32_t*)(blob + L.fstat))[f] = frag_status[f];
        }
        float* mpos = (float*)(blob + L.mpos) + 3 * (size_t)fr.o_mv;
        const float* sp = A.pos + 3 * (size_t)fr.mv_off;
        for (uint32_t i = tid; i < 3 * fr.mv_n; i += group_size()) mpos[i] = sp[i];
        uint32_t* mno = (uint32_t*)(blob + L.mno) + fr.o_mv;
        for (uint32_t v = tid; v < fr.mv_n; v += group_size()) mno[v] = fr.o_mh + (A.loff[fr.mv_off + v] - fr.mh_off);
        int32_t* mnbr = (int32_t*)(blob + L.mnbr) + fr.o_mh;
        for (uint32_t e = tid; e < fr.mh_n; e += group_size()) mnbr[e] = A.nbr[fr.mh_off + e];
        float* cpos = (float*)(blob + L.cpos) + 3 * (size_t)fr.o_cv;
        const float* scp = A.pos + 3 * (size_t)fr.cv_off;
        for (uint32_t i = tid; i < 3 * fr.cv_n; i += group_size()) cpos[i] = scp[i];
        uint32_t* cno = (uint32_t*)(blob + L.cno) + fr.o_cv;
        for (uint32_t v = tid; v < fr.cv_n; v += group_size()) cno[v] = fr.o_ch + (A.loff[fr.cv_off + v] - fr.ch_off);
        int32_t* cnbr = (int32_t*)(blob + L.cnbr) + fr.o_ch;
        for (uint32_t e = tid; e < fr.ch_n; e += group_size()) cnbr[e] = A.nbr[fr.ch_off + e];
        if (with_vnc)
        {
            float* vnc = (float*)(blob + L.vnc) + 9 * (size_t)fr.o_mv;
            for (uint32_t i = tid; i < 9 * fr.mv_n; i += group_size())
            {
                const uint32_t v = i / 9, k = i % 9;
                vnc[i] = k < 3 ? sp[3 * v + k] : (k < 6 ? 0.f : (k == 6 ? cr : (k == 7 ? cg : cb)));
            }
        }
        uint32_t* idx = (uint32_t*)(blob + L.idx) + fr.o_idx;
        for (uint32_t e = tid; e < fr.idx_n; e += group_size()) idx[e] = A.idx[fr.idx_off + e];
    }
}

__global__ __launch_bounds__(SURTR_WG) void k_clip_single(SolidIn in, const float4* __restrict__ planes, uint32_t F,
                                                          ScratchPool pool, float* opos, uint32_t* ooff, int32_t* onbr,
                                                          uint32_t* ollen, uint32_t cap_v, uint32_t cap_h,
                                                          uint32_t* result )
{
    __shared__ Shared sh;
    __shared__ LdsTopo L;
    Scratch S = carve(pool, 0);
    for (uint32_t k = threadIdx.x; k < F; k += group_size()) sh.planes[k] = planes[k];
    __syncthreads();
    uint32_t n = 0, nh = 0;
    int err = SURTR_E_TOPOLOGY;
    if (in.nv > SURTR_LITERAL_MESH_V || !solid_is_sliver(in))
        err = clip_any(in, F, S, sh, L, [&](auto& T) -> int {
            if (T.nLive == 0) return 0;
            const uint2 tot = index_live(T, sh);
            if (tot.x > cap_v || tot.y > cap_h) return SURTR_E_CAPACITY;
            write_solid(T, opos, ooff, ollen, onbr, 0, 0);
            n = tot.x; nh = tot.y;
            return 0;
        });
    __syncthreads();
    if (err == SURTR_E_TOPOLOGY)
    {
        const LitRun r = literal_run(in, F, pool, 0, &sh);
        if (r.err == 0 && (r.n > cap_v || r.nh > cap_h)) err = SURTR_E_CAPACITY;
        else if (r.err == 0) { literal_write(r, opos, ooff, ollen, onbr, 0, 0); n = r.n; nh = r.nh; err = 0; }
        else if (r.err != SURTR_E_TOPOLOGY) err = r.err;
    }
    if (threadIdx.x == 0) { if (err == 0) ooff[n] = nh; result[0] = n; result[1] = nh; result[2] = (uint32_t)err; }
}


extern "C" {

const char* surtr_strerror(int code)
{
    switch (code)
    {
    case SURTR_OK: return "ok";
    case SURTR_E_INVALID: return "invalid argument";
    case SURTR_E_TOPOLOGY: return "topology error (asymmetric links or degree < 3)";
    case SURTR_E_CAPACITY: return "capacity exceeded";
    case SURTR_E_HIP: return "HIP runtime error";
    case SURTR_E_STATE: return "call order violated";
    case SURTR_E_NOGPU: return "no HIP device (the engine has no CPU fallback)";
    default: return "unknown";
    }
}

int surtr_create(int device, surtr_ctx** out)
{
    if (!out) return SURTR_E_INVALID;
    *out = nullptr;
    int n = 0;
    if (hipGetDeviceCount(&n) != hipSuccess || n <= 0) return SURTR_E_NOGPU;
    if (device < 0 || device >= n) return SURTR_E_INVALID;
    if (hipSetDevice(device) != hipSuccess) return SURTR_E_HIP;
    surtr_ctx* ctx = new surtr_ctx;
    ctx->device = device;
    {
        hipDeviceProp_t prop;
        if (hipGetDeviceProperties(&prop, device) == hipSuccess && prop.multiProcessorCount > 0)
        {
            uint32_t per_cu = 2u;
            if (const char* e = getenv("SURTR_WG_PER_CU")) { const int v = atoi(e); if (v > 0 && v <= 32) per_cu = (uint32_t)v; }
            ctx->max_wg = (uint32_t)prop.multiProcessorCount * per_cu;
            ctx->max_wg_faces = (uint32_t)prop.multiProcessorCount * 4u;
            uint32_t half_per_cu = 4u;
            if (const char* e = getenv("SURTR_HALF_PER_CU")) { const int v = atoi(e); if (v > 0 && v <= 32) half_per_cu = (uint32_t)v; }
            ctx->max_wg_half = (uint32_t)prop.multiProcessorCount * half_per_cu;
            uint32_t small_per_cu = 8u;
            if (const char* e = getenv("SURTR_SMALL_PER_CU")) { const int v = atoi(e); if (v > 0 && v <= 32) small_per_cu = (uint32_t)v; }
            ctx->max_wg_small = (uint32_t)prop.multiProcessorCount * small_per_cu;
            uint32_t prep_per_cu = SURTR_PREP_WAVES;
            if (const char* e = getenv("SURTR_PREP_PER_CU")) { const int v = atoi(e); if (v > 0 && v <= 32) prep_per_cu = (uint32_t)v; }
            ctx->max_wg_prep = (uint32_t)prop.multiProcessorCount * prep_per_cu;
        }
        ctx->hw_wg = ctx->max_wg; ctx->hw_wg_faces = ctx->max_wg_faces; ctx->hw_wg_prep = ctx->max_wg_prep; ctx->hw_wg_big = ctx->n_wg_big;
    }
    if (ctx->d_counts.grow(ctx, 1) != SURTR_OK || ctx->arena_buf.cursors.grow(ctx, CUR_COUNT) != SURTR_OK ||
        hipStreamCreateWithFlags(&ctx->stream2, hipStreamNonBlocking) != hipSuccess ||
        hipStreamCreateWithFlags(&ctx->stream3, hipStreamNonBlocking) != hipSuccess ||
        hipEventCreateWithFlags(&ctx->ev_half, hipEventDisableTiming) != hipSuccess ||
        hipEventCreateWithFlags(&ctx->ev_cvx, hipEventDisableTiming) != hipSuccess ||
        hipEventCreateWithFlags(&ctx->ev_prep, hipEventDisableTiming) != hipSuccess ||
        hipEventCreateWithFlags(&ctx->ev_big, hipEventDisableTiming) != hipSuccess) { surtr_destroy(ctx); return SURTR_E_HIP; }
    ctx->arena.cursors = ctx->arena_buf.cursors;
    if (const char* e = getenv("SURTR_EVENTS_IN_FLIGHT")) { const int v = atoi(e); if (v > 0) ctx->events_in_flight = (uint32_t)v; }
    *out = ctx;
    return SURTR_OK;
}

void surtr_regroup_forget(const surtr_ctx* ctx);

void surtr_destroy(surtr_ctx* ctx)
{
    if (!ctx) return;
    surtr_regroup_forget(ctx);
    (void)hipSetDevice(ctx->device);
    (void)hipDeviceSynchronize();
    if (ctx->stream2) (void)hipStreamDestroy(ctx->stream2);
    if (ctx->stream3) (void)hipStreamDestroy(ctx->stream3);
    if (ctx->ev_half) (void)hipEventDestroy(ctx->ev_half);
    if (ctx->ev_cvx) (void)hipEventDestroy(ctx->ev_cvx);
    if (ctx->ev_prep) (void)hipEventDestroy(ctx->ev_prep);
    if (ctx->ev_big) (void)hipEventDestroy(ctx->ev_big);
    for (int i = 0; i < 32; ++i) if (ctx->ev[i]) (void)hipEventDestroy(ctx->ev[i]);
    for (int i = 0; i < 16; ++i) for (int q = 0; q < 2; ++q) if (ctx->hev[i][q]) (void)hipEventDestroy(ctx->hev[i][q]);
    delete ctx;
}

const char* surtr_last_error(surtr_ctx* ctx) { return ctx ? ctx->err.c_str() : ""; }

int surtr_set_stream(surtr_ctx* ctx, void* s)
{
    if (!ctx) return SURTR_E_INVALID;
    ctx->stream = (hipStream_t)s;
    return SURTR_OK;
}

int surtr_get_stream(surtr_ctx* ctx, void** s)
{
    if (!ctx || !s) return SURTR_E_INVALID;
    *s = (void*)ctx->stream;
    return SURTR_OK;
}

static void free_scratch(surtr_ctx* ctx);
static void free_arena(surtr_ctx* ctx);

int surtr_set_scratch(surtr_ctx* ctx, uint32_t mv, uint32_t mh)
{
    if (!ctx) return SURTR_E_INVALID;
    ctx->user_cv = mv; ctx->user_ch = mh;
    free_scratch(ctx);
    return SURTR_OK;
}

int surtr_set_arena(surtr_ctx* ctx, uint64_t v, uint64_t h, uint64_t i)
{
    if (!ctx) return SURTR_E_INVALID;
    ctx->user_av = v; ctx->user_ah = h; ctx->user_ai = i;
    free_arena(ctx);
    return SURTR_OK;
}

static int check_solid(uint32_t nv, const uint32_t* off, const int32_t* nbr)
{
    for (uint32_t v = 0; v < nv; ++v)
    {
        if (off[v + 1] < off[v]) return SURTR_E_INVALID;
        const uint32_t deg = off[v + 1] - off[v];
        if (deg < 3) return SURTR_E_TOPOLOGY;
        for (uint32_t j = off[v]; j < off[v + 1]; ++j)
        {
            const int32_t u = nbr[j];
            if (u < 0 || (uint32_t)u >= nv || (uint32_t)u == v) return SURTR_E_TOPOLOGY;
            bool back = false;
            for (uint32_t q = off[u]; q < off[u + 1]; ++q) if (nbr[q] == (int32_t)v) { back = true; break; }
            if (!back) return SURTR_E_TOPOLOGY;
        }
    }
    return SURTR_OK;
}

int surtr_upload_pattern(surtr_ctx* ctx, uint32_t n_cells, const uint32_t* face_off, const float* v012)
{
    if (!ctx || n_cells == 0 || !face_off || !v012) return SURTR_E_INVALID;
    (void)hipSetDevice(ctx->device);
    const uint32_t nf = face_off[n_cells];
    for (uint32_t c = 0; c < n_cells; ++c)
        if (face_off[c + 1] < face_off[c] || face_off[c + 1] - face_off[c] > SURTR_MAXF) return SURTR_E_INVALID;
    ctx->planes_ready = false;
    ctx->d_v012.reset(); ctx->d_planes.reset(); ctx->d_plane_off.reset();
    int rc = ctx->d_v012.grow(ctx, std::max<size_t>(4, (size_t)nf * 9));
    if (rc == SURTR_OK) rc = ctx->d_planes.grow(ctx, std::max(nf, 1u));
    if (rc == SURTR_OK) rc = ctx->d_plane_off.grow(ctx, (size_t)n_cells + 1);
    if (rc) { ctx->d_v012.reset(); ctx->d_planes.reset(); return rc; }
    HIPCHK(hipMemcpy(ctx->d_v012, v012, (size_t)nf * 36, hipMemcpyHostToDevice));
    HIPCHK(hipMemcpy(ctx->d_plane_off, face_off, (size_t)(n_cells + 1) * 4, hipMemcpyHostToDevice));
    ctx->h_plane_off.assign(face_off, face_off + n_cells + 1);
    ctx->n_cells = n_cells; ctx->n_faces = nf; ctx->planes_ready = false; ctx->pair_order_count = 0;
    return SURTR_OK;
}

int surtr_place_cells(surtr_ctx* ctx, const float scale[3], const float translate[3])
{
    if (!ctx || !scale || !translate) return SURTR_E_INVALID;
    if (!ctx->d_v012) return SURTR_E_STATE;
    (void)hipSetDevice(ctx->device);
    const uint32_t nf = ctx->n_faces;
    if (nf)
        hipLaunchKernelGGL(k_place_cells, dim3((nf + 255) / 256), dim3(256), 0, ctx->stream, nf, ctx->d_v012, scale[0], scale[1],
                           scale[2], translate[0], translate[1], translate[2], ctx->d_planes);
    HIPCHK(hipGetLastError());
    ctx->planes_ready = true;
    return SURTR_OK;
}

int surtr_upload_planes(surtr_ctx* ctx, uint32_t n_cells, const uint32_t* plane_off, const float* planes)
{
    if (!ctx || n_cells == 0 || !plane_off || !planes) return SURTR_E_INVALID;
    (void)hipSetDevice(ctx->device);
    const uint32_t nf = plane_off[n_cells];
    for (uint32_t c = 0; c < n_cells; ++c)
        if (plane_off[c + 1] < plane_off[c] || plane_off[c + 1] - plane_off[c] > SURTR_MAXF) return SURTR_E_INVALID;
    ctx->planes_ready = false;
    ctx->d_v012.reset(); ctx->d_planes.reset(); ctx->d_plane_off.reset();
    int rc = ctx->d_planes.grow(ctx, std::max(nf, 1u));
    if (rc == SURTR_OK) rc = ctx->d_plane_off.grow(ctx, (size_t)n_cells + 1);
    if (rc) { ctx->d_planes.reset(); return rc; }
    HIPCHK(hipMemcpy(ctx->d_planes, planes, (size_t)nf * 16, hipMemcpyHostToDevice));
    HIPCHK(hipMemcpy(ctx->d_plane_off, plane_off, (size_t)(n_cells + 1) * 4, hipMemcpyHostToDevice));
    ctx->h_plane_off.assign(plane_off, plane_off + n_cells + 1);
    ctx->n_cells = n_cells; ctx->n_faces = nf; ctx->planes_ready = true; ctx->pair_order_count = 0;
    return SURTR_OK;
}

#define SURTR_FACES_TIER_DEFAULT 524288u
static void budget_workgroups(surtr_ctx* ctx)
{
    if (ctx->budget_vmax == ctx->vmax && ctx->budget_hmax == ctx->hmax) return;
    ctx->budget_vmax = ctx->vmax; ctx->budget_hmax = ctx->hmax;
    size_t free_b = 0, total_b = 0;
    if (hipMemGetInfo(&free_b, &total_b) != hipSuccess || total_b == 0) total_b = (size_t)64 << 30;
    if (const char* e = getenv("SURTR_MEM_BUDGET_MB")) { const long v = atol(e); if (v > 0) total_b = (size_t)v << 20; }
    auto fit = [](size_t budget, size_t per, uint32_t lo, uint32_t hi) {
        const size_t n = per ? budget / per : hi;
        return (uint32_t)std::min<size_t>(hi, std::max<size_t>(lo, n));
    };
    const uint32_t CV = ctx->user_cv ? ctx->user_cv : 2 * ctx->vmax + 4096, CH = ctx->user_ch ? ctx->user_ch : 3 * ctx->hmax + 16384;
    const uint32_t all = fit(total_b / 4, scratch_bytes_per_wg(std::max(CV, 64u), CH, ctx->vmax), 20u, ctx->hw_wg + std::max(ctx->hw_wg / 2u, ctx->hw_wg_big));
    ctx->wave_big = ctx->vmax >= 80000u && ctx->vmax < 300000u;
    if (const char* e = getenv("SURTR_WAVE_BIG")) ctx->wave_big = atoi(e) != 0;
    const uint32_t hw_big = ctx->wave_big ? std::max(ctx->hw_wg / 2u, ctx->hw_wg_big) : ctx->hw_wg_big;
    ctx->n_wg_big = all >= ctx->hw_wg + hw_big ? hw_big : std::min(hw_big, std::max(4u, all / 8u));
    ctx->max_wg = std::min(ctx->hw_wg, all - ctx->n_wg_big);
    size_t HF = (size_t)ctx->hmax + ctx->hmax / 2 + 8192;
    {
        size_t tier = SURTR_FACES_TIER_DEFAULT;
        if (const char* e = getenv("SURTR_FACES_TIER_HE")) { const long v = atol(e); if (v >= 64) tier = (size_t)v; }
        HF = std::min(HF, tier);
    }
    ctx->max_wg_faces = fit(total_b / 8, HF * 48, 16u, ctx->hw_wg_faces);
    ctx->max_wg_prep = fit(total_b / 16, prep_bytes_per_wg(std::max(ctx->vmax, 64u)), 16u, ctx->hw_wg_prep);
}

static int alloc_pool(surtr_ctx* ctx, DevBuf<char>& buf, ScratchPool& view, uint32_t& view_wg, uint32_t CV, uint32_t CH, uint32_t VMAX, uint32_t n_wg)
{
    view = ScratchPool{}; view_wg = 0;
    buf.reset();
    const ScratchPool P{nullptr, scratch_bytes_per_wg(CV, CH, VMAX), CV, CH, VMAX};
    const int rc = buf.grow(ctx, P.per_wg * n_wg);
    if (rc) return rc;
    view = P; view.base = buf; view_wg = n_wg;
    return SURTR_OK;
}

static void free_scratch(surtr_ctx* ctx)
{
    ctx->pool_buf.reset(); ctx->fs_buf.reset(); ctx->d_blk.reset(); ctx->fs_big_buf.reset(); ctx->d_blk_big.reset();
    ctx->pool = ScratchPool{}; ctx->fs = FaceScratch{}; ctx->fs_big = FaceScratch{};
    ctx->n_wg = ctx->n_wg_faces_alloc = ctx->n_wg_faces_big = ctx->blk_per_wg = ctx->blk_per_wg_big = 0;
}

static int ensure_scratch(surtr_ctx* ctx, uint32_t need_v, uint32_t need_h, uint32_t n_wg)
{
    uint32_t n_wg_faces = std::max(1u, ctx->max_wg_faces);
    if (const char* e = getenv("SURTR_FACES_WG")) { const uint32_t v = (uint32_t)atoi(e); if (v > n_wg_faces && v <= 8192u) n_wg_faces = v; }
    uint32_t CV = ctx->user_cv ? ctx->user_cv : 2 * need_v + 4096;
    uint32_t CH = ctx->user_ch ? ctx->user_ch : 3 * need_h + 16384;
    if (CV < 64) CV = 64;
    const uint32_t VMAX = need_v;
    if (ctx->pool.base && ctx->pool.CV >= CV && ctx->pool.CH >= CH && ctx->pool.VMAX >= VMAX && ctx->n_wg >= n_wg && ctx->n_wg_faces_alloc >= n_wg_faces) return SURTR_OK;
    free_scratch(ctx);
    int rc = alloc_pool(ctx, ctx->pool_buf, ctx->pool, ctx->n_wg, CV, CH, VMAX, n_wg);
    const uint32_t HF_full = need_h + need_h / 2 + 8192;
    uint32_t tier = SURTR_FACES_TIER_DEFAULT;
    if (ctx->events_in_flight > 1u) tier /= 4u;
    if (const char* e = getenv("SURTR_FACES_TIER_HE")) { const long v = atol(e); if (v >= 64) tier = (uint32_t)v; }
    FaceScratch fs{nullptr, 0, std::min(HF_full, tier)};
    fs.per_wg = (size_t)12 * fs.HF;
    const uint32_t blk_per_wg = fs.HF / SURTR_LANES + 4;
    if (rc == SURTR_OK) rc = ctx->fs_buf.grow(ctx, fs.per_wg * n_wg_faces);
    if (rc == SURTR_OK) rc = ctx->d_blk.grow(ctx, (size_t)blk_per_wg * n_wg_faces);
    FaceScratch fs_big{}; uint32_t n_wg_big = 0, blk_per_wg_big = 0;
    if (rc == SURTR_OK && HF_full > fs.HF)
    {
        size_t free_b = 0, total_b = 0;
        if (hipMemGetInfo(&free_b, &total_b) != hipSuccess || total_b == 0) total_b = (size_t)64 << 30;
        if (const char* e = getenv("SURTR_MEM_BUDGET_MB")) { const long v = atol(e); if (v > 0) total_b = (size_t)v << 20; }
        fs_big.HF = HF_full; fs_big.per_wg = (size_t)12 * HF_full;
        n_wg_big = (uint32_t)std::min<size_t>(64, std::max<size_t>(2, (total_b / 16) / (fs_big.per_wg * 4)));
        blk_per_wg_big = HF_full / SURTR_LANES + 4;
        rc = ctx->fs_big_buf.grow(ctx, fs_big.per_wg * n_wg_big);
        if (rc == SURTR_OK) rc = ctx->d_blk_big.grow(ctx, (size_t)blk_per_wg_big * n_wg_big);
    }
    if (rc) { free_scratch(ctx); return rc; }
    fs.base = ctx->fs_buf; fs_big.base = ctx->fs_big_buf;
    ctx->fs = fs; ctx->blk_per_wg = blk_per_wg; ctx->n_wg_faces_alloc = n_wg_faces;
    ctx->fs_big = fs_big; ctx->blk_per_wg_big = blk_per_wg_big; ctx->n_wg_faces_big = n_wg_big;
    return SURTR_OK;
}

static int ensure_scratch_small(surtr_ctx* ctx, uint32_t n_wg)
{
    const uint32_t need_v = 2 * ctx->cvmax + 4 * SURTR_MAXF + 256, need_h = 2 * ctx->chmax + 12 * SURTR_MAXF + 1024;
    const uint32_t CV = 2 * need_v + 1024, CH = 3 * need_h + 4096, VMAX = need_v;
    if (ctx->pool_small.base && ctx->pool_small.CV >= CV && ctx->pool_small.CH >= CH && ctx->n_wg_small >= n_wg) return SURTR_OK;
    return alloc_pool(ctx, ctx->pool_small_buf, ctx->pool_small, ctx->n_wg_small, CV, CH, VMAX, n_wg);
}

static int ensure_scratch_half(surtr_ctx* ctx, uint32_t n_wg)
{
    if (ctx->pool_half.base && ctx->n_wg_half >= n_wg) return SURTR_OK;
    return alloc_pool(ctx, ctx->pool_half_buf, ctx->pool_half, ctx->n_wg_half, SURTR_LVS + 256u, SURTR_LHS + 256u, SURTR_LVS + 64u, n_wg);
}

static int ensure_prep(surtr_ctx* ctx, uint32_t n_pairs, uint32_t n_wg)
{
    const uint32_t VMAX = std::max(ctx->vmax, 64u);
    if (!(ctx->prep.base && ctx->prep.VMAX >= VMAX && ctx->n_wg_prep >= n_wg))
    {
        ctx->prep = PrepPool{nullptr, 0, 0}; ctx->n_wg_prep = 0;
        ctx->prep_buf.reset();
        const size_t per_wg = prep_bytes_per_wg(VMAX);
        const int rc = ctx->prep_buf.grow(ctx, per_wg * n_wg);
        if (rc) return rc;
        ctx->prep = PrepPool{ctx->prep_buf, per_wg, VMAX}; ctx->n_wg_prep = n_wg;
    }
    int rc = ctx->d_order.grow(ctx, (size_t)n_pairs * 64);
    if (rc) return rc;
    const uint64_t full = (uint64_t)ctx->vmax * 16 + (uint64_t)ctx->hmax * 2;
    const uint64_t lds = (uint64_t)SURTR_LV * 16 + (uint64_t)SURTR_LH * 2;
    const uint64_t per_pair = std::min(full, lds) + ctx->vmax / 8 + 2048;
    uint64_t bytes = std::min<uint64_t>(std::max<uint64_t>((uint64_t)n_pairs * per_pair, 1ull << 20), 4ull << 30);
    if (const char* e = getenv("SURTR_IMG_BYTES")) { const long long v = atoll(e); if (v >= 4096) bytes = (uint64_t)v; }
    const uint32_t cap16 = (uint32_t)(bytes / 16);
    if (!(ctx->img.base && ctx->img.cap16 >= cap16) || (getenv("SURTR_IMG_BYTES") && ctx->img.cap16 != cap16))
    {
        ctx->img = ImgArena{nullptr, 0};
        ctx->img_buf.reset();
        rc = ctx->img_buf.grow(ctx, (size_t)cap16 * 16);
        if (rc) return rc;
        ctx->img = ImgArena{ctx->img_buf, cap16};
    }
    return SURTR_OK;
}

static void free_arena(surtr_ctx* ctx)
{
    auto& B = ctx->arena_buf;
    B.pos.reset(); B.loff.reset(); B.llen.reset(); B.nbr.reset(); B.idx.reset(); B.isl.reset();
    ctx->d_frags.reset(); ctx->d_forder.reset(); ctx->d_frag_status.reset(); ctx->d_face_list.reset();
    ctx->arena = Arena{}; ctx->arena.cursors = B.cursors; ctx->cap_frags = 0;
}

static uint32_t refit_planes(const surtr_ctx* ctx) { return std::min(2u * RH_MAXFACE, 2u * (3u * ctx->refit_limit - 8u)); }

static int ensure_arena(surtr_ctx* ctx, uint32_t n_pairs, uint64_t min_v = 0, uint64_t min_h = 0, uint64_t min_i = 0)
{
    const uint64_t xp = refit_planes(ctx) - 8u;
    uint64_t av = ctx->user_av ? ctx->user_av : std::max<uint64_t>(std::max<uint64_t>((uint64_t)ctx->vmax * 8, ctx->tot_mv * 3) + (uint64_t)n_pairs * (256 + 8 * xp), 1u << 16);
    uint64_t ah = ctx->user_ah ? ctx->user_ah : std::max<uint64_t>(std::max<uint64_t>((uint64_t)ctx->hmax * 8, ctx->tot_mh * 3) + (uint64_t)n_pairs * (1024 + 32 * xp), 1u << 18);
    uint64_t ai = ctx->user_ai ? ctx->user_ai : ah * 2;
    av = std::max(av, min_v); ah = std::max(ah, min_h); ai = std::max(ai, min_i);
    av = std::min<uint64_t>(av, 0xFFFFFFF0ull); ah = std::min<uint64_t>(ah, 0xFFFFFFF0ull); ai = std::min<uint64_t>(ai, 0xFFFFFFF0ull);
    const uint32_t capIsl = (uint32_t)std::min<uint64_t>((uint64_t)n_pairs * 4 + 1024, 0x7FFFFFFFull);
    if (!(ctx->arena.pos && ctx->arena.capV >= av && ctx->arena.capH >= ah && ctx->arena.capI >= ai && ctx->arena.capIsl >= capIsl))
    {
        free_arena(ctx);
        auto& B = ctx->arena_buf;
        int rc = B.pos.grow(ctx, av * 3);
        if (rc == SURTR_OK) rc = B.loff.grow(ctx, av);
        if (rc == SURTR_OK) rc = B.llen.grow(ctx, av);
        if (rc == SURTR_OK) rc = B.nbr.grow(ctx, ah);
        if (rc == SURTR_OK) rc = B.idx.grow(ctx, ai);
        if (rc == SURTR_OK) rc = B.isl.grow(ctx, capIsl);
        if (rc == SURTR_OK) rc = ctx->d_frags.grow(ctx, capIsl);
        if (rc == SURTR_OK) rc = ctx->d_forder.grow(ctx, (size_t)capIsl * 16);
        if (rc == SURTR_OK) rc = ctx->d_frag_status.grow(ctx, capIsl);
        if (rc == SURTR_OK) rc = ctx->d_face_list.grow(ctx, capIsl);
        if (rc) { free_arena(ctx); return rc; }
        ctx->arena = Arena{B.pos, B.loff, B.llen, B.nbr, B.idx, B.isl, (uint32_t)av, (uint32_t)ah, (uint32_t)ai, capIsl, B.cursors};
        ctx->cap_frags = capIsl;
    }
    const int rc = ctx->d_pairs.grow(ctx, n_pairs);
    if (rc) return rc;
    return ctx->d_scanblk.grow(ctx, std::max(n_pairs, ctx->cap_frags) / SURTR_LANES + 4);
}

__global__ void k_event_init(uint32_t* __restrict__ cursors, uint32_t* __restrict__ counts, uint32_t n_counts, uint32_t* __restrict__ frag_status,
                             uint32_t n_status, uint32_t* __restrict__ hlist, uint32_t n_hlist)
{
    const uint32_t i0 = blockIdx.x * blockDim.x + threadIdx.x, step = gridDim.x * blockDim.x;
    for (uint32_t i = i0; i < CUR_COUNT; i += step) cursors[i] = 0u;
    for (uint32_t i = i0; i < n_counts; i += step) counts[i] = 0u;
    for (uint32_t i = i0; i < n_status; i += step) frag_status[i] = 0u;
    for (uint32_t i = i0; i < n_hlist; i += step) hlist[i] = 0xFFFFFFFFu;
}

static int upload_pair_order(surtr_ctx* ctx, const uint32_t* ord, uint32_t n_pairs)
{
    const int rc = ctx->d_pair_order.grow(ctx, n_pairs);
    if (rc) return rc;
    HIPCHK(hipStreamSynchronize(ctx->stream));
    HIPCHK(hipMemcpyAsync(ctx->d_pair_order, ord, (size_t)n_pairs * 4, hipMemcpyHostToDevice, ctx->stream));
    HIPCHK(hipStreamSynchronize(ctx->stream));
    return SURTR_OK;
}

#ifndef SURTR_REC_MAXN
#define SURTR_REC_MAXN 2304u
#endif
#ifndef SURTR_FRONT_PAR_MAX
#define SURTR_FRONT_PAR_MAX 1024u
#endif
struct EventPlan
{
    bool cell_order;
    decltype(&k_prep_pairs) prep;
    uint32_t prep_threads;
    bool wave_on, split_on, use_half, front_par, both;
    uint32_t rec_on;
    uint32_t big_quota, big_n, walk0, n_catch, n_poll;
    uint32_t n_wg, n_wg_cvx, n_wg_prep, n_wg_big, n_wg_half, n_wg_retry, n_wg_sweep;
    uint32_t g_refit, g_faces, t_faces;
    hipStream_t st_cvx, st_main, st_bigk, st_refit;
};

static EventPlan plan_event(const surtr_ctx* ctx, uint32_t n_pairs, bool pair_list, uint32_t flags)
{
    EventPlan pl{};
    const uint32_t n1 = std::max(n_pairs, 1u), max_wg = ctx->max_wg;
    pl.cell_order = !pair_list && n_pairs && ctx->n_pieces && n_pairs % ctx->n_pieces == 0 && !getenv("SURTR_NO_CELL_ORDER");
    pl.n_wg = std::max(1u, std::min(n1, max_wg));
    pl.n_wg_cvx = std::max(1u, std::min(n1, ctx->max_wg_small));
    pl.n_wg_half = std::max(1u, std::min(n1, ctx->max_wg_half));
    pl.n_wg_prep = std::max(1u, std::min(n1, ctx->max_wg_prep));
    pl.n_wg_big = std::min(ctx->n_wg_big, n1);
    pl.n_wg_retry = std::min(pl.n_wg, 64u);
    pl.big_quota = ctx->wave_big ? 0xFFFFFFFFu : 2u * ctx->n_wg_big;
    if (const char* e = getenv("SURTR_BIG_QUOTA")) pl.big_quota = (uint32_t)atoi(e);
    pl.big_n = (ctx->wave_big && ctx->vmax < 180000u) ? 2800u : 0xFFFFFFFFu;
    const bool half_forced = getenv("SURTR_HALF") != nullptr && atoi(getenv("SURTR_HALF")) != 0;
    const bool many = ctx->events_in_flight > 1u && !half_forced;
    pl.wave_on = 2u * n_pairs > 3u * max_wg || (!half_forced && ctx->vmin >= SURTR_PREP_MINV && ctx->vmax <= 4u * SURTR_REC_MAXN) ||
                 (many && ctx->vmin >= SURTR_PREP_MINV && ctx->vmax <= ctx->prep.VMAX);
    if (const char* e = getenv("SURTR_WAVE")) pl.wave_on = atoi(e) != 0;
    pl.rec_on = pl.wave_on ? 1u : 0u;
    if (const char* e = getenv("SURTR_REC")) pl.rec_on = (pl.wave_on && atoi(e) != 0) ? 1u : 0u;
    if (const char* e = getenv("SURTR_PREP_SORTED")) { if (atoi(e) == 0) pl.rec_on = 2u; }
    uint32_t rec_maxn = SURTR_REC_MAXN;
    if (const char* e = getenv("SURTR_REC_MAXN")) rec_maxn = (uint32_t)atoi(e);
    pl.rec_on |= (rec_maxn < 0xFFFFFFu ? rec_maxn : 0xFFFFFFu) << 8;
    pl.split_on = pl.wave_on && ctx->vmin >= SURTR_PREP_MINV && ctx->vmax <= ctx->prep.VMAX;
    if (const char* e = getenv("SURTR_SPLIT")) pl.split_on = pl.split_on && atoi(e) != 0;
    pl.use_half = ctx->half_on && (!pl.split_on || half_forced);
    pl.n_catch = std::min(SURTR_CATCH_WG_MAX, n1);
    pl.n_wg_sweep = std::min(pl.n_catch, SURTR_CATCH_POLL);
    pl.n_poll = ctx->events_in_flight > 1u ? 2u : SURTR_CATCH_POLL;
    if (const char* e = getenv("SURTR_CATCH_POLL")) { const int v = atoi(e); if (v >= 0 && v <= 1024) pl.n_poll = (uint32_t)v; }
    uint32_t wide_max = 4u * ctx->max_wg;
    if (const char* e = getenv("SURTR_PREP_WIDE_MAX")) wide_max = (uint32_t)atoi(e);
    const bool prep_wide = n_pairs != 0 && n_pairs <= wide_max && ctx->vmax >= 8192u && !many;
    pl.front_par = n_pairs != 0 && n_pairs <= SURTR_FRONT_PAR_MAX && !prep_wide;
    if (const char* e = getenv("SURTR_FRONT_PAR")) pl.front_par = n_pairs != 0 && atoi(e) != 0;
    if (pl.front_par) pl.rec_on |= 4u;
    pl.prep = nullptr; pl.prep_threads = SURTR_WG;
    if (n_pairs && prep_wide) { pl.prep = k_prep_pairs_wide; pl.prep_threads = SURTR_WG_WIDE; }
    else if (n_pairs && !(pl.rec_on & 2u) && ctx->vmax < 0xFFFFu && ctx->vmin >= SURTR_PREP_MINV && (ctx->vmax + SURTR_LANES - 1u) / SURTR_LANES <= SURTR_PREP_NB)
        pl.prep = k_prep_pairs_sorted;
    else if (n_pairs) pl.prep = k_prep_pairs;
    pl.walk0 = SURTR_WWALK0;
    if (const char* e = getenv("SURTR_WWALK0")) { const int v = atoi(e); if (v >= 0 && v <= 64) pl.walk0 = (uint32_t)v; }
    pl.st_cvx = pl.front_par ? ctx->stream3 : ctx->stream;
    pl.st_main = pl.front_par ? ctx->stream : ctx->stream2;
    pl.st_bigk = pl.front_par ? ctx->stream2 : ctx->stream;
    pl.both = (flags & SURTR_EVT_REFIT) && (flags & SURTR_EVT_RENDER);
    pl.st_refit = pl.both ? ctx->stream2 : ctx->stream;
    pl.g_refit = ctx->n_wg_small;
    if (pl.both) pl.g_refit = std::min(pl.g_refit, ctx->max_wg_faces / 4u * 5u);
    if (pl.both) if (const char* e = getenv("SURTR_REFIT_WG_BOTH")) { const uint32_t v = (uint32_t)atoi(e); if (v > 0 && v <= ctx->n_wg_small) pl.g_refit = v; }
    pl.g_faces = std::max(1u, ctx->max_wg_faces); pl.t_faces = SURTR_WG;
    if (pl.both) pl.g_faces = std::max(1u, ctx->max_wg_faces / 2u);
    if (pl.both) if (const char* e = getenv("SURTR_FACES_WG_BOTH")) { const uint32_t v = (uint32_t)atoi(e); if (v > 0 && v <= ctx->n_wg_faces_alloc) pl.g_faces = v; }
    if (const char* e = getenv("SURTR_FACES_WG")) { const uint32_t v = (uint32_t)atoi(e); if (v > 0 && v <= ctx->n_wg_faces_alloc) pl.g_faces = v; }
    if (const char* e = getenv("SURTR_FACES_THREADS")) { const uint32_t v = (uint32_t)atoi(e); if (v == 64 || v == 128 || v == 256) pl.t_faces = v; }
    return pl;
}

static int ensure_hull_ws(surtr_ctx* ctx)
{
    if (ctx->refit_limit <= 4u || ctx->d_hull_ws.cap >= 2 * (size_t)ctx->arena.capV) return SURTR_OK;
    HIPCHK(hipStreamSynchronize(ctx->stream));
    return ctx->d_hull_ws.grow(ctx, 2 * (size_t)ctx->arena.capV);
}

static void launch_refit(surtr_ctx* ctx, uint32_t grid, hipStream_t st, bool of_pieces)
{
    const float* cpos = of_pieces ? (const float*)ctx->cset.pos : (const float*)nullptr;
    const uint32_t* cvo = of_pieces ? (const uint32_t*)ctx->cset.vo : (const uint32_t*)nullptr;
    if (ctx->refit_limit <= 4u)
        hipLaunchKernelGGL(k_refit, dim3(grid), dim3(SURTR_LANES), 0, st, ctx->d_frags, ctx->d_counts, ctx->pool_small, ctx->arena, ctx->d_forder, ctx->cap_frags, ctx->d_frag_status,
                           cpos, cvo);
    else
        hipLaunchKernelGGL(k_refit_n, dim3(grid), dim3(SURTR_LANES), 0, st, ctx->d_frags, ctx->d_counts, ctx->pool_small, ctx->arena, ctx->d_forder, ctx->cap_frags, ctx->d_frag_status,
                           cpos, cvo, ctx->refit_limit, (uint32_t*)ctx->d_hull_ws);
}

static int launch_event(surtr_ctx* ctx, uint32_t cell_begin, uint32_t n_pairs, const uint2* d_pair_list, const uint8_t* outside, uint32_t flags)
{
    (void)hipSetDevice(ctx->device);
    budget_workgroups(ctx);
    const uint32_t max_wg = ctx->max_wg, n1 = std::max(n_pairs, 1u);
    int rc = ensure_scratch(ctx, ctx->vmax, ctx->hmax, max_wg + ctx->n_wg_big + SURTR_CATCH_WG_MAX);
    if (rc) return rc;
    rc = ensure_scratch_small(ctx, std::max(ctx->max_wg_small, ctx->n_wg_small));
    if (rc) return rc;
    rc = ensure_scratch_half(ctx, std::max(ctx->max_wg_half, ctx->n_wg_half));
    if (rc) return rc;
    rc = ensure_arena(ctx, n1);
    if (rc) return rc;
    if (flags & SURTR_EVT_REFIT) { rc = ensure_hull_ws(ctx); if (rc) return rc; }
    rc = ensure_prep(ctx, n1, std::max(std::max(1u, std::min(n1, ctx->max_wg_prep)), ctx->n_wg_prep));
    if (rc) return rc;
    hipStream_t st = ctx->stream, st2 = ctx->stream2, st3 = ctx->stream3;
    const uint32_t hcap = n_pairs + 4096u;
    if (ctx->d_hlist.cap < hcap)
    {
        HIPCHK(hipStreamSynchronize(st));
        rc = ctx->d_hlist.grow(ctx, hcap);
        if (rc) return rc;
    }
    const EventPlan pl = plan_event(ctx, n_pairs, d_pair_list != nullptr, flags);
    static_assert(sizeof(surtr_counts) % 4 == 0, "surtr_counts is cleared by words");
    hipLaunchKernelGGL(k_event_init, dim3(SURTR_LANES == 1 ? 1 : 64), dim3(SURTR_LANES == 1 ? 1 : 256), 0, st, ctx->arena.cursors, (uint32_t*)ctx->d_counts.p,
                       (uint32_t)(sizeof(surtr_counts) / 4), ctx->d_frag_status, ctx->cap_frags, ctx->d_hlist, hcap);
    const uint8_t* d_out = nullptr;
    ctx->last_outside.clear();
    if (outside) ctx->last_outside.assign(outside, outside + ctx->n_pieces);
    if (outside)
    {
        HIPCHK(hipMemcpyAsync(ctx->d_outside, outside, ctx->n_pieces, hipMemcpyHostToDevice, st));
        d_out = ctx->d_outside;
    }
    const PieceSet& M = ctx->mset; const PieceSet& C = ctx->cset;
    Pieces P{M.pos, M.loff, M.llen, M.nbr, M.vo, M.tri, M.rad, M.perm, M.posr_s, M.bsph, M.bo,
             C.pos, C.loff, C.llen, C.nbr, C.vo, C.tri, C.rad, C.perm, C.posr_s, C.bsph, C.bo, ctx->n_pieces, M.dup, C.dup,
             M.row_s, M.iperm, M.bsph2, M.bo2, M.bsph3, M.bo3};
    for (int i = 0; i < 16; ++i) ctx->ev_valid[i] = false;
    const uint32_t* d_pair_order = nullptr;
    if (d_pair_list && ctx->pair_order_is_list && ctx->pair_order_count == n_pairs) d_pair_order = ctx->d_pair_order;
    else if (pl.cell_order)
    {
        const uint32_t np = ctx->n_pieces, nc = n_pairs / np;
        if (ctx->pair_order_is_list || ctx->pair_order_begin != cell_begin || ctx->pair_order_count != n_pairs)
        {
            std::vector<uint32_t> cells(nc), ord((size_t)n_pairs);
            for (uint32_t i = 0; i < nc; ++i) cells[i] = i;
            const std::vector<uint32_t>& po = ctx->h_plane_off;
            std::stable_sort(cells.begin(), cells.end(), [&](uint32_t a, uint32_t b) {
                return po[cell_begin + a + 1] - po[cell_begin + a] > po[cell_begin + b + 1] - po[cell_begin + b]; });
            for (uint32_t i = 0; i < nc; ++i) for (uint32_t q = 0; q < np; ++q) ord[(size_t)i * np + q] = cells[i] * np + q;
            int rc2 = upload_pair_order(ctx, ord.data(), n_pairs);
            if (rc2) return rc2;
            ctx->pair_order_is_list = false; ctx->pair_order_begin = cell_begin; ctx->pair_order_count = n_pairs;
        }
        d_pair_order = ctx->d_pair_order;
    }
    uint32_t* const order = ctx->d_order;
    const size_t cap_order = ctx->d_order.cap / 64;
    uint32_t* const porder = ctx->d_order + 16 * cap_order;
    uint32_t* const horder = ctx->d_order + 32 * cap_order;
    const bool wave = n_pairs && pl.wave_on, split = wave && pl.split_on;

    if (pl.front_par)
    {
        HIPCHK(hipEventRecord(ctx->ev_prep, st));
        HIPCHK(hipStreamWaitEvent(pl.st_cvx, ctx->ev_prep, 0));
    }
    PROF_BEGIN_ON(6, pl.st_cvx);
    if (n_pairs)
        hipLaunchKernelGGL(k_clip_convex, dim3(pl.n_wg_cvx), dim3(SURTR_LANES), 0, pl.st_cvx, P, ctx->d_planes, ctx->d_plane_off, cell_begin, n_pairs,
                           d_out, ctx->pool_small, ctx->arena, ctx->d_pairs, d_pair_list, pl.front_par ? (uint32_t*)nullptr : porder, d_pair_order,
                           pl.front_par ? 1u : 0u);
    PROF_END_ON(6, pl.st_cvx);
    if (pl.front_par) HIPCHK(hipEventRecord(ctx->ev_cvx, pl.st_cvx));
    PROF_BEGIN(7);
    if (pl.prep)
        hipLaunchKernelGGL(pl.prep, dim3(pl.n_wg_prep), dim3(pl.prep_threads), 0, st, P, ctx->d_planes, ctx->d_plane_off, cell_begin, n_pairs,
                           ctx->prep, ctx->arena, ctx->img, std::min((uint32_t)SURTR_LV, ctx->pool.CV), std::min((uint32_t)SURTR_LVS, ctx->pool_half.CV),
                           ctx->d_pairs, d_pair_list, order, porder, horder, pl.use_half ? 1u : 0u, pl.big_quota, pl.big_n, pl.rec_on);
    PROF_END(7);
    HIPCHK(hipEventRecord(ctx->ev_prep, st));
    HIPCHK(hipStreamWaitEvent(st2, ctx->ev_prep, 0));
    HIPCHK(hipStreamWaitEvent(st3, ctx->ev_prep, 0));
    if (pl.front_par)
    {
        HIPCHK(hipStreamWaitEvent(st, ctx->ev_cvx, 0));
        HIPCHK(hipStreamWaitEvent(st2, ctx->ev_cvx, 0));
    }
    PROF_BEGIN_ON(8, pl.st_bigk);
    if (n_pairs && ctx->wave_big)
        hipLaunchKernelGGL(k_clip_pairs_wave_big, dim3(pl.n_wg_big), dim3(SURTR_WG), 0, pl.st_bigk, P, ctx->d_planes,
                           ctx->d_plane_off, cell_begin, n_pairs, ctx->pool, max_wg, ctx->arena, ctx->img, ctx->d_pairs, d_pair_list, order, 15, 14, CUR_Q_BIG, pl.walk0);
    else if (n_pairs)
        hipLaunchKernelGGL(k_clip_pairs_big, dim3(pl.n_wg_big), dim3(SURTR_WG), 0, pl.st_bigk, P, ctx->d_planes,
                           ctx->d_plane_off, cell_begin, n_pairs, ctx->pool, max_wg, ctx->arena, ctx->img, ctx->d_pairs, d_pair_list, order);
    PROF_END_ON(8, pl.st_bigk);
    PROF_BEGIN_ON(11, pl.st_main);
    if (wave) PROF_HIST_BEGIN(11, pl.st_main);
    if (split)
        hipLaunchKernelGGL(k_clip_pairs_main, dim3(pl.n_wg), dim3(SURTR_MAIN_THREADS), 0, pl.st_main, P, ctx->d_planes, ctx->d_plane_off, cell_begin, n_pairs,
                           ctx->pool, ctx->arena, ctx->img, ctx->d_pairs, d_pair_list, order, ctx->d_hlist, pl.walk0);
    else if (wave)
        hipLaunchKernelGGL(k_clip_pairs_wave, dim3(pl.n_wg), dim3(SURTR_WG), 0, pl.st_main, P, ctx->d_planes, ctx->d_plane_off, cell_begin, n_pairs,
                           ctx->pool, ctx->arena, ctx->img, ctx->d_pairs, d_pair_list, order, horder, 13, 0, CUR_Q_CLIP, pl.walk0);
    if (wave) PROF_HIST_END(11, pl.st_main);
    PROF_END_ON(11, pl.st_main);
    PROF_BEGIN_ON(0, pl.st_main);
    if (n_pairs && !pl.wave_on)
    {
        PROF_HIST_BEGIN(0, pl.st_main);
        hipLaunchKernelGGL(k_clip_pairs, dim3(pl.n_wg), dim3(SURTR_WG), 0, pl.st_main, P, ctx->d_planes, ctx->d_plane_off, cell_begin, n_pairs,
                           ctx->pool, ctx->arena, ctx->img, ctx->d_pairs, d_pair_list, order, horder, 13, 0, CUR_Q_CLIP);
        PROF_HIST_END(0, pl.st_main);
    }
    PROF_END_ON(0, pl.st_main);
    PROF_BEGIN_ON(13, st3);
    if (split)
        hipLaunchKernelGGL(k_clip_pairs_catch, dim3(pl.n_catch), dim3(SURTR_WG), 0, st3, P, ctx->d_planes, ctx->d_plane_off, cell_begin, n_pairs,
                           ctx->pool, max_wg + ctx->n_wg_big, ctx->arena, ctx->img, ctx->d_pairs, d_pair_list, order, ctx->d_hlist, hcap, pl.n_wg, 0u, pl.n_poll);
    PROF_END_ON(13, st3);
    PROF_BEGIN_ON(9, st3);
    if (n_pairs && pl.use_half)
        hipLaunchKernelGGL(k_clip_pairs_half, dim3(pl.n_wg_half), dim3(SURTR_WGS), 0, st3, P, ctx->d_planes, ctx->d_plane_off, cell_begin, n_pairs,
                           ctx->pool_half, ctx->arena, ctx->img, ctx->d_pairs, d_pair_list, horder);
    PROF_END_ON(9, st3);
    HIPCHK(hipEventRecord(ctx->ev_half, st3));
    HIPCHK(hipStreamWaitEvent(pl.st_main, ctx->ev_half, 0));
    PROF_BEGIN_ON(10, pl.st_main);
    if (n_pairs && pl.use_half)
        hipLaunchKernelGGL(k_clip_pairs, dim3(pl.n_wg_retry), dim3(SURTR_WG), 0, pl.st_main, P, ctx->d_planes, ctx->d_plane_off, cell_begin, n_pairs,
                           ctx->pool, ctx->arena, ctx->img, ctx->d_pairs, d_pair_list, order, horder, -1, 0, CUR_Q_RETRY);
    if (split)
        hipLaunchKernelGGL(k_clip_pairs_catch, dim3(pl.n_wg_sweep), dim3(SURTR_WG), 0, pl.st_main, P, ctx->d_planes, ctx->d_plane_off, cell_begin, n_pairs,
                           ctx->pool, max_wg + ctx->n_wg_big, ctx->arena, ctx->img, ctx->d_pairs, d_pair_list, order, ctx->d_hlist, hcap, pl.n_wg, 1u, 0u);
    PROF_END_ON(10, pl.st_main);
    HIPCHK(hipEventRecord(ctx->ev_big, st2));
    HIPCHK(hipStreamWaitEvent(st, ctx->ev_big, 0));
    PROF_BEGIN(1);
    hipLaunchKernelGGL(k_frag_table, dim3(1), dim3(SURTR_WG_WIDE), 0, st, ctx->d_pairs, n_pairs, ctx->n_pieces, cell_begin, ctx->arena,
                       ctx->d_scanblk, ctx->d_frags, ctx->cap_frags, ctx->d_counts, d_pair_list, ctx->d_forder);
    PROF_END(1);
    if (pl.both)
    {
        HIPCHK(hipEventRecord(ctx->ev_prep, st));
        HIPCHK(hipStreamWaitEvent(pl.st_refit, ctx->ev_prep, 0));
    }
    if (flags & SURTR_EVT_REFIT)
    {
        PROF_BEGIN_ON(2, pl.st_refit);
        launch_refit(ctx, pl.g_refit, pl.st_refit, true);
        PROF_END_ON(2, pl.st_refit);
    }
    if (flags & SURTR_EVT_RENDER)
    {
        PROF_BEGIN(3);
        const bool tiers = ctx->n_wg_faces_big != 0;
        hipLaunchKernelGGL(k_faces, dim3(pl.g_faces), dim3(pl.t_faces), 0, st, ctx->d_frags, ctx->d_counts, ctx->fs, ctx->d_blk,
                           ctx->blk_per_wg, ctx->arena, ctx->d_forder, ctx->cap_frags, 0u, (uint32_t*)nullptr, (uint32_t*)nullptr, (int32_t*)nullptr,
                           ctx->d_frag_status, (const uint32_t*)nullptr, tiers ? ctx->d_face_list : (uint32_t*)nullptr);
        if (tiers)
            hipLaunchKernelGGL(k_faces, dim3(ctx->n_wg_faces_big), dim3(pl.t_faces), 0, st, ctx->d_frags, ctx->d_counts, ctx->fs_big, ctx->d_blk_big,
                               ctx->blk_per_wg_big, ctx->arena, ctx->d_forder, ctx->cap_frags, 0u, (uint32_t*)nullptr, (uint32_t*)nullptr, (int32_t*)nullptr,
                               ctx->d_frag_status, (const uint32_t*)ctx->d_face_list, (uint32_t*)nullptr);
        PROF_END(3);
    }
    if (pl.both)
    {
        HIPCHK(hipEventRecord(ctx->ev_big, st2));
        HIPCHK(hipStreamWaitEvent(st, ctx->ev_big, 0));
    }
    PROF_BEGIN(4);
    hipLaunchKernelGGL(k_out_scan, dim3(1), dim3(SURTR_WG_WIDE), 0, st, ctx->d_frags, ctx->d_scanblk, ctx->d_counts, ctx->arena);
    PROF_END(4);
    HIPCHK(hipGetLastError());
    ctx->have_event = true; ctx->last_flags = flags; ctx->last_current = false; ctx->frags_of_pieces = true;
    ctx->scene_event_compound = -1;
    return SURTR_OK;
}

int surtr_fracture_event_async(surtr_ctx* ctx, uint32_t cell_begin, uint32_t cell_end, const uint8_t* outside, uint32_t flags)
{
    if (!ctx) return SURTR_E_INVALID;
    if (!ctx->n_pieces || !ctx->planes_ready) return SURTR_E_STATE;
    if (cell_end > ctx->n_cells || cell_begin > cell_end) return SURTR_E_INVALID;
    return launch_event(ctx, cell_begin, (cell_end - cell_begin) * ctx->n_pieces, nullptr, outside, flags);
}

int surtr_fracture_pairs_async(surtr_ctx* ctx, uint32_t n_pairs, const uint32_t* pair_cell, const uint32_t* pair_piece, uint32_t flags)
{
    return surtr_event_pairs_masked(ctx, n_pairs, pair_cell, pair_piece, nullptr, flags);
}

}

int surtr_event_pairs_masked(surtr_ctx* ctx, uint32_t n_pairs, const uint32_t* pair_cell, const uint32_t* pair_piece, const uint8_t* outside, uint32_t flags)
{
    if (!ctx || (n_pairs && (!pair_cell || !pair_piece))) return SURTR_E_INVALID;
    if (!ctx->n_pieces || !ctx->planes_ready) return SURTR_E_STATE;
    (void)hipSetDevice(ctx->device);
    std::vector<uint2> list(n_pairs);
    for (uint32_t i = 0; i < n_pairs; ++i)
    {
        if (pair_cell[i] >= ctx->n_cells || pair_piece[i] >= ctx->n_pieces) return SURTR_E_INVALID;
        list[i].x = pair_cell[i]; list[i].y = pair_piece[i];
    }
    const int rc = ctx->d_pair_list.grow(ctx, std::max(n_pairs, 1u));
    if (rc) return rc;
    if (n_pairs) HIPCHK(hipMemcpyAsync(ctx->d_pair_list, list.data(), (size_t)n_pairs * sizeof(uint2), hipMemcpyHostToDevice, ctx->stream));
    HIPCHK(hipStreamSynchronize(ctx->stream));
    ctx->pair_order_count = 0;
    if (n_pairs && !getenv("SURTR_NO_CELL_ORDER"))
    {
        const std::vector<uint32_t>& po = ctx->h_plane_off;
        uint32_t start[SURTR_MAXF + 2] = {0};
        for (uint32_t i = 0; i < n_pairs; ++i) ++start[SURTR_MAXF - (po[pair_cell[i] + 1] - po[pair_cell[i]]) + 1];
        for (uint32_t k = 1; k <= SURTR_MAXF + 1; ++k) start[k] += start[k - 1];
        std::vector<uint32_t> ord(n_pairs);
        for (uint32_t i = 0; i < n_pairs; ++i) ord[start[SURTR_MAXF - (po[pair_cell[i] + 1] - po[pair_cell[i]])]++] = i;
        int rc2 = upload_pair_order(ctx, ord.data(), n_pairs);
        if (rc2) return rc2;
        ctx->pair_order_is_list = true; ctx->pair_order_count = n_pairs;
    }
    return launch_event(ctx, 0, n_pairs, ctx->d_pair_list, outside, flags);
}

extern "C" {

int surtr_place_cells_groups_dev(surtr_ctx* ctx, uint32_t n_groups, const uint32_t* group_cell_off, const float* d_scale3, const float* d_shift3)
{
    if (!ctx || !n_groups || !group_cell_off || !d_scale3 || !d_shift3) return SURTR_E_INVALID;
    if (!ctx->d_v012) return SURTR_E_STATE;
    if (group_cell_off[0] != 0 || group_cell_off[n_groups] != ctx->n_cells) return SURTR_E_INVALID;
    (void)hipSetDevice(ctx->device);
    const uint32_t nf = ctx->n_faces;
    std::vector<uint32_t> face_group(std::max(nf, 1u));
    for (uint32_t g = 0; g < n_groups; ++g)
    {
        if (group_cell_off[g + 1] < group_cell_off[g]) return SURTR_E_INVALID;
        for (uint32_t c = group_cell_off[g]; c < group_cell_off[g + 1]; ++c)
            for (uint32_t f = ctx->h_plane_off[c]; f < ctx->h_plane_off[c + 1]; ++f) face_group[f] = g;
    }
    const int rc = ctx->d_face_group.grow(ctx, std::max(nf, 1u), (size_t)nf + nf / 4 + 64);
    if (rc) return rc;
    HIPCHK(hipMemcpyAsync(ctx->d_face_group, face_group.data(), (size_t)nf * 4, hipMemcpyHostToDevice, ctx->stream));
    if (nf)
        hipLaunchKernelGGL(k_place_cells_groups, dim3((nf + 255) / 256), dim3(256), 0, ctx->stream, nf, ctx->d_v012, ctx->d_face_group, d_scale3, d_shift3, ctx->d_planes);
    HIPCHK(hipGetLastError());
    HIPCHK(hipStreamSynchronize(ctx->stream));
    ctx->planes_ready = true;
    return SURTR_OK;
}

int surtr_place_cells_groups(surtr_ctx* ctx, uint32_t n_groups, const uint32_t* group_cell_off, const float* scale3, const float* translate3)
{
    if (!ctx || !n_groups || !group_cell_off || !scale3 || !translate3) return SURTR_E_INVALID;
    (void)hipSetDevice(ctx->device);
    DevBuf<float> d;
    const int rc = d.grow(ctx, (size_t)n_groups * 6);
    if (rc) return rc;
    HIPCHK(hipMemcpy(d, scale3, (size_t)n_groups * 12, hipMemcpyHostToDevice));
    HIPCHK(hipMemcpy(d + 3 * (size_t)n_groups, translate3, (size_t)n_groups * 12, hipMemcpyHostToDevice));
    return surtr_place_cells_groups_dev(ctx, n_groups, group_cell_off, d, d + 3 * (size_t)n_groups);
}

int surtr_event_refit(surtr_ctx* ctx)
{
    if (!ctx) return SURTR_E_INVALID;
    if (!ctx->have_event) return SURTR_E_STATE;
    (void)hipSetDevice(ctx->device);
    hipStream_t st = ctx->stream;
    const int rc = ensure_hull_ws(ctx);
    if (rc) return rc;
    HIPCHK(hipMemsetAsync(ctx->arena.cursors + CUR_Q_REFIT, 0, 4, st));
    PROF_BEGIN(2);
    launch_refit(ctx, ctx->n_wg_small, st, ctx->frags_of_pieces);
    PROF_END(2);
    hipLaunchKernelGGL(k_out_scan, dim3(1), dim3(SURTR_WG_WIDE), 0, st, ctx->d_frags, ctx->d_scanblk, ctx->d_counts, ctx->arena);
    HIPCHK(hipGetLastError());
    ctx->last_flags |= SURTR_EVT_REFIT; ctx->last_current = false;
    return SURTR_OK;
}

static int launch_faces(surtr_ctx* ctx, uint32_t fan, uint32_t* d_face_n, uint32_t* d_face_off, int32_t* d_face_idx)
{
    hipStream_t st = ctx->stream;
    HIPCHK(hipMemsetAsync(ctx->arena.cursors + CUR_Q_FACES, 0, 4, st));
    HIPCHK(hipMemsetAsync(ctx->arena.cursors + CUR_I, 0, 4, st));
    if (!(ctx->last_flags & SURTR_EVT_REFIT))
    {
        HIPCHK(hipMemsetAsync(ctx->arena.cursors + CUR_FLAGGED_FRAGS, 0, 4, st));
        HIPCHK(hipMemsetAsync(ctx->d_frag_status, 0, (size_t)ctx->cap_frags * 4, st));
    }
    PROF_BEGIN(3);
    const bool tiers = ctx->n_wg_faces_big != 0;
    if (tiers) HIPCHK(hipMemsetAsync(ctx->arena.cursors + CUR_FACES2_N, 0, 8, st));
    hipLaunchKernelGGL(k_faces, dim3(std::max(1u, ctx->max_wg_faces)), dim3(SURTR_WG), 0, st, ctx->d_frags, ctx->d_counts, ctx->fs, ctx->d_blk,
                       ctx->blk_per_wg, ctx->arena, ctx->d_forder, ctx->cap_frags, fan, d_face_n, d_face_off, d_face_idx, ctx->d_frag_status,
                       (const uint32_t*)nullptr, tiers ? ctx->d_face_list : (uint32_t*)nullptr);
    if (tiers)
        hipLaunchKernelGGL(k_faces, dim3(ctx->n_wg_faces_big), dim3(SURTR_WG), 0, st, ctx->d_frags, ctx->d_counts, ctx->fs_big, ctx->d_blk_big,
                           ctx->blk_per_wg_big, ctx->arena, ctx->d_forder, ctx->cap_frags, fan, d_face_n, d_face_off, d_face_idx, ctx->d_frag_status,
                           (const uint32_t*)ctx->d_face_list, (uint32_t*)nullptr);
    PROF_END(3);
    hipLaunchKernelGGL(k_out_scan, dim3(1), dim3(SURTR_WG_WIDE), 0, st, ctx->d_frags, ctx->d_scanblk, ctx->d_counts, ctx->arena);
    HIPCHK(hipGetLastError());
    ctx->last_flags |= SURTR_EVT_RENDER; ctx->last_current = false;
    return SURTR_OK;
}

int surtr_event_triangulate(surtr_ctx* ctx, int is_convex)
{
    if (!ctx) return SURTR_E_INVALID;
    if (!ctx->have_event) return SURTR_E_STATE;
    (void)hipSetDevice(ctx->device);
    return launch_faces(ctx, is_convex ? 1u : 0u, nullptr, nullptr, nullptr);
}

int surtr_load_fragments(surtr_ctx* ctx, uint32_t n, const uint32_t* mvo, const float* mpos, const uint32_t* moff, const int32_t* mnbr,
                         const uint32_t* cvo, const float* cpos, const uint32_t* coff, const int32_t* cnbr, const int32_t* frag_ids)
{
    if (!ctx || n == 0 || !mvo || !mpos || !moff || !mnbr || !cvo || !cpos || !coff || !cnbr) return SURTR_E_INVALID;
    (void)hipSetDevice(ctx->device);
    const uint32_t MV = mvo[n], CV = cvo[n];
    const uint32_t MH = moff[MV], CH = coff[CV];
    uint32_t vmax = 0, hmax = 0, cvmax = 0, chmax = 0;
    for (uint32_t k = 0; k < n; ++k)
    {
        for (int set = 0; set < 2; ++set)
        {
            const uint32_t* vo = set ? cvo : mvo; const uint32_t* off = set ? coff : moff; const int32_t* nbr = set ? cnbr : mnbr;
            const uint32_t a = vo[k], b = vo[k + 1];
            if (b < a || b - a < 4) return SURTR_E_INVALID;
            std::vector<uint32_t> loc(b - a + 1);
            for (uint32_t v = a; v <= b; ++v) loc[v - a] = off[v] - off[a];
            const int rc = check_solid(b - a, loc.data(), nbr + off[a]);
            if (rc) return rc;
            if (set) { cvmax = std::max(cvmax, b - a); chmax = std::max(chmax, off[b] - off[a]); }
            else { vmax = std::max(vmax, b - a); hmax = std::max(hmax, off[b] - off[a]); }
        }
    }
    ctx->cvmax = std::max(ctx->cvmax, cvmax); ctx->chmax = std::max(ctx->chmax, chmax);
    ctx->vmax = std::max(ctx->vmax, std::max(vmax, cvmax)); ctx->hmax = std::max(ctx->hmax, std::max(hmax, chmax));
    int rc = ensure_scratch(ctx, ctx->vmax, ctx->hmax, std::max(1u, ctx->n_wg));
    if (rc) return rc;
    rc = ensure_scratch_small(ctx, std::max(ctx->max_wg_small, ctx->n_wg_small));
    if (rc) return rc;
    const uint64_t rp = refit_planes(ctx);
    rc = ensure_arena(ctx, n, (uint64_t)MV + 3ull * CV + 8ull * rp * n, (uint64_t)MH + 4ull * CH + 32ull * rp * n, 3ull * MH + 64);
    if (rc) return rc;
    if (n > ctx->cap_frags) return SURTR_E_CAPACITY;
    hipStream_t st = ctx->stream;
    HIPCHK(hipStreamSynchronize(st));
    std::vector<uint32_t> loff((size_t)MV + CV), llen((size_t)MV + CV);
    for (uint32_t v = 0; v < MV; ++v) { loff[v] = moff[v]; llen[v] = moff[v + 1] - moff[v]; }
    for (uint32_t v = 0; v < CV; ++v) { loff[MV + v] = MH + coff[v]; llen[MV + v] = coff[v + 1] - coff[v]; }
    std::vector<FragRec> fr(n);
    std::vector<uint32_t> cursors(CUR_STATS_WORDS, 0u), forder((size_t)16 * ctx->cap_frags, 0u);
    for (uint32_t k = 0; k < n; ++k)
    {
        FragRec& r = fr[k];
        memset(&r, 0, sizeof(r));
        r.cell = frag_ids ? frag_ids[3 * k] : (int32_t)k; r.piece = frag_ids ? frag_ids[3 * k + 1] : 0; r.island = frag_ids ? frag_ids[3 * k + 2] : 0;
        r.mv_off = mvo[k]; r.mv_n = mvo[k + 1] - mvo[k]; r.mh_off = moff[mvo[k]]; r.mh_n = moff[mvo[k + 1]] - moff[mvo[k]];
        r.cv_off = MV + cvo[k]; r.cv_n = cvo[k + 1] - cvo[k]; r.ch_off = MH + coff[cvo[k]]; r.ch_n = coff[cvo[k + 1]] - coff[cvo[k]];
        uint32_t cls = 0; while ((r.mv_n >> (cls + 1u)) != 0u && cls < 15u) ++cls;
        forder[(size_t)cls * ctx->cap_frags + cursors[CUR_CLS_FRAG + cls]++] = k;
    }
    cursors[CUR_V] = MV + CV; cursors[CUR_H] = MH + CH;
    surtr_counts c; memset(&c, 0, sizeof(c)); c.n_frag = n; c.n_pairs = n;
    HIPCHK(hipMemcpyAsync(ctx->arena.pos, mpos, (size_t)MV * 12, hipMemcpyHostToDevice, st));
    HIPCHK(hipMemcpyAsync(ctx->arena.pos + 3 * (size_t)MV, cpos, (size_t)CV * 12, hipMemcpyHostToDevice, st));
    HIPCHK(hipMemcpyAsync(ctx->arena.loff, loff.data(), loff.size() * 4, hipMemcpyHostToDevice, st));
    HIPCHK(hipMemcpyAsync(ctx->arena.llen, llen.data(), llen.size() * 4, hipMemcpyHostToDevice, st));
    HIPCHK(hipMemcpyAsync(ctx->arena.nbr, mnbr, (size_t)MH * 4, hipMemcpyHostToDevice, st));
    HIPCHK(hipMemcpyAsync(ctx->arena.nbr + MH, cnbr, (size_t)CH * 4, hipMemcpyHostToDevice, st));
// ... 416 lines not shown
```

Baseline: 1.133 million.

## Add lean convex-clip kernel with compact LDS and giveup fallback pass

Templates the small-clip LDS structures over capacity and word width, so a lean kernel can run with a smaller LDS footprint and more waves per CU. The lean kernel handles most convex pairs and queues those it cannot handle into a giveup list. A second, small launch of the full k_clip_convex then processes only that list. The goal is higher occupancy for the common case, at the cost of an extra launch, a serialized tail pass, and extra atomics.

```diff
diff --git a/surtr_amd/csrc/small_clip.h b/surtr_amd/csrc/small_clip.h
--- a/surtr_amd/csrc/small_clip.h
+++ b/surtr_amd/csrc/small_clip.h
@@ -7,29 +7,43 @@
 
 namespace surtr {
 
-struct ScSolid
-{
-    float pos[3 * SC_V];
-    uint32_t vw[SC_V];
-    uint32_t re[SC_H];
+template <uint32_t CAPV, uint32_t CAPH, class WORD = uint32_t>
+struct ScSolidT
+{
+    typedef WORD Word;
+    static constexpr uint32_t kVwSh = sizeof(WORD) == 4 ? 16u : 12u, kReSh = sizeof(WORD) == 4 ? 16u : 8u;
+    static_assert(CAPV <= (1u << kReSh) && CAPH <= (1u << kVwSh), "a vertex id / a ring offset fits its field");
+    float pos[3 * CAPV];
+    WORD vw[CAPV];
+    WORD re[CAPH];
 };
-
-struct ScLds
-{
-    ScSolid buf[2];
-    int8_t c[SC_V];
-    uint16_t km[SC_V];
-    uint16_t mp[SC_V];
-    uint16_t noff[SC_V];
-    uint16_t succ[SC_V], pred[SC_V];
+typedef ScSolidT<SC_V, SC_H> ScSolid;
+
+template <uint32_t CAPV, uint32_t CAPH, class WORD = uint32_t>
+struct ScLdsT
+{
+    static_assert(CAPV % 4u == 0 && CAPV <= 0x7FFFu && CAPH <= 0xFFFFu, "16-bit indices, 4-byte arrays");
+    static constexpr uint32_t kV = CAPV, kH = CAPH;
+    typedef ScSolidT<CAPV, CAPH, WORD> Solid;
+    Solid buf[2];
+    int8_t c[CAPV];
+    uint16_t km[CAPV];
+    uint16_t mp[CAPV];
+    uint16_t noff[CAPV];
+    uint16_t succ[CAPV], pred[CAPV];
     uint32_t nv[2], flag;
 #ifdef SURTR_STAMP
     unsigned long long tph[8];
 #endif
 };
-
-__device__ inline int small_clip(const SolidIn in, const uint32_t F, const Shared& sh, ScLds& L, uint32_t* which, uint32_t* stop = nullptr)
-{
+typedef ScLdsT<SC_V, SC_H> ScLds;
+
+template <class SH, class LDS>
+__device__ inline int small_clip(const SolidIn in, const uint32_t F, const SH& sh, LDS& L, uint32_t* which, uint32_t* stop = nullptr)
+{
+    typedef typename LDS::Solid ScSolid;
+    constexpr uint32_t CAPV = LDS::kV, CAPH = LDS::kH;
+    constexpr uint32_t VS = ScSolid::kVwSh, VM = (1u << VS) - 1u, RS = ScSolid::kReSh, RM = (1u << RS) - 1u;
     const uint32_t lane = lane_id();
     const uint32_t V = in.nv;
 #ifdef SURTR_STAMP
@@ -40,9 +54,9 @@
 #define SC_STAMP(i) do { } while (0)
 #endif
     if (stop != nullptr) *stop = 0xFFFFFFFFu;
-    if (V == 0 || V > SC_V) return SC_FALLBACK;
+    if (V == 0 || V > CAPV) return SC_FALLBACK;
     const uint32_t hbase = in.loff[0], H = in.loff[V - 1u] + in.llen[V - 1u] - hbase;
-    if (H > SC_H) return SC_FALLBACK;
+    if (H > CAPH) return SC_FALLBACK;
     bool odd = false;
     for (uint32_t v = lane; v < V; v += SURTR_LANES)
     {
@@ -51,12 +65,12 @@
         const uint32_t lo = in.loff[v] - hbase, deg = in.llen[v];
         if (deg > 15u || deg < 3u) odd = true;
         const uint32_t dl = deg > 15u ? 15u : deg;
-        S.vw[v] = lo | (dl << 16);
+        S.vw[v] = lo | (dl << VS);
         const int32_t* r = in.nbr + in.loff[v];
-        for (uint32_t j = 0; j < dl && lo + j < SC_H; ++j)
+        for (uint32_t j = 0; j < dl && lo + j < CAPH; ++j)
         {
             if ((uint32_t)r[j] >= V) odd = true;
-            S.re[lo + j] = (uint32_t)r[j] & 0xFFFFu;
+            S.re[lo + j] = (uint32_t)r[j] & RM;
             for (uint32_t jj = 0; jj < j; ++jj) if (r[jj] == r[j]) odd = true;
         }
     }
@@ -65,15 +79,15 @@
     for (uint32_t v = lane; v < V; v += SURTR_LANES)
     {
         ScSolid& S = L.buf[0];
-        const uint32_t w = S.vw[v], lo = w & 0xFFFFu, deg = w >> 16;
+        const uint32_t w = S.vw[v], lo = w & VM, deg = w >> VS;
         for (uint32_t j = 0; j < deg; ++j)
         {
-            const uint32_t e = S.re[lo + j] & 0xFFFFu;
-            const uint32_t we = S.vw[e], elo = we & 0xFFFFu, edeg = we >> 16;
+            const uint32_t e = S.re[lo + j] & RM;
+            const uint32_t we = S.vw[e], elo = we & VM, edeg = we >> VS;
             uint32_t q = 0;
-            while (q < edeg && (S.re[elo + q] & 0xFFFFu) != v) ++q;
+            while (q < edeg && (S.re[elo + q] & RM) != v) ++q;
             if (q >= edeg) odd = true;
-            S.re[lo + j] = e | (q << 16);
+            S.re[lo + j] = e | (q << RS);
         }
     }
     if (__ballot(odd) != 0ull) return SC_FALLBACK;
@@ -105,11 +119,11 @@
             uint32_t mask = 0, isKept = 0, deg = 0;
             if (v < nv)
             {
-                const uint32_t w = S.vw[v], lo = w & 0xFFFFu;
-                deg = w >> 16;
+                const uint32_t w = S.vw[v], lo = w & VM;
+                deg = w >> VS;
                 if (L.c[v] > 0) isKept = 1u;
                 else
-                    for (uint32_t j = 0; j < deg; ++j) if (L.c[S.re[lo + j] & 0xFFFFu] > 0) mask |= 1u << j;
+                    for (uint32_t j = 0; j < deg; ++j) if (L.c[S.re[lo + j] & RM] > 0) mask |= 1u << j;
             }
             const uint32_t cnt = (uint32_t)__builtin_popcount(mask);
             const uint2 inc = wave_incl_scan2(make_uint2(cnt | (isKept << 16), isKept ? deg : 0u));
@@ -123,7 +137,7 @@
             carryM += tx & 0xFFFFu; carryK += tx >> 16; carryH += ty;
         }
         const uint32_t M = carryM, nKeep = carryK, HK = carryH;
-        if (nKeep + M > SC_V || HK + 3u * M > SC_H) SC_GIVE_UP;
+        if (nKeep + M > CAPV || HK + 3u * M > CAPH) SC_GIVE_UP;
         if (nKeep + M < 4u) { nv = 0; break; }
         for (uint32_t t = lane; t < M; t += SURTR_LANES) L.pred[t] = 0xFFFFu;
         __syncthreads();
@@ -140,12 +154,12 @@
                 uint32_t cv = v, w = wv, slot = (uint32_t)__builtin_ctz(mask), steps = 0, end = 0xFFFFu;
                 while (steps++ <= nv)
                 {
-                    const uint32_t len = w >> 16;
+                    const uint32_t len = w >> VS;
                     const uint32_t p = slot == 0u ? len - 1u : slot - 1u;
-                    const uint32_t rw = S.re[(w & 0xFFFFu) + p];
-                    const uint32_t e = rw & 0xFFFFu;
+                    const uint32_t rw = S.re[(w & VM) + p];
+                    const uint32_t e = rw & RM;
                     if (L.c[e] > 0) { end = (L.mp[cv] & 0x7FFFu) + (uint32_t)__builtin_popcount(L.km[cv] & ((1u << p) - 1u)); break; }
-                    cv = e; slot = rw >> 16; w = S.vw[e];
+                    cv = e; slot = rw >> RS; w = S.vw[e];
                 }
                 if (end == 0xFFFFu || end == t) { bad = true; continue; }
                 L.succ[t] = (uint16_t)end;
@@ -160,18 +174,18 @@
         SC_STAMP(4);
         for (uint32_t v = lane; v < nv; v += SURTR_LANES)
         {
-            const uint32_t w = S.vw[v], lo0 = w & 0xFFFFu, deg = w >> 16;
+            const uint32_t w = S.vw[v], lo0 = w & VM, deg = w >> VS;
             if (L.c[v] > 0)
             {
                 const uint32_t id = L.mp[v], lo = L.noff[v];
                 N.pos[3 * id] = S.pos[3 * v]; N.pos[3 * id + 1] = S.pos[3 * v + 1]; N.pos[3 * id + 2] = S.pos[3 * v + 2];
-                N.vw[id] = lo | (deg << 16);
+                N.vw[id] = lo | (deg << VS);
                 for (uint32_t j = 0; j < deg; ++j)
                 {
-                    const uint32_t rw = S.re[lo0 + j], e = rw & 0xFFFFu, q = rw >> 16;
+                    const uint32_t rw = S.re[lo0 + j], e = rw & RM, q = rw >> RS;
                     const uint32_t m = L.mp[e], kme = L.km[e];
-                    N.re[lo + j] = (m & 0x8000u) ? (nKeep + (m & 0x7FFFu) + (uint32_t)__builtin_popcount(kme & ((1u << q) - 1u))) | (2u << 16)
-                                                 : m | (q << 16);
+                    N.re[lo + j] = (m & 0x8000u) ? (nKeep + (m & 0x7FFFu) + (uint32_t)__builtin_popcount(kme & ((1u << q) - 1u))) | (2u << RS)
+                                                 : m | (q << RS);
                 }
             }
             else
@@ -181,7 +195,7 @@
                 uint32_t t = L.mp[v] & 0x7FFFu;
                 for (uint32_t mask = L.km[v]; mask; mask &= mask - 1u, ++t)
                 {
-                    const uint32_t rw = S.re[lo0 + (uint32_t)__builtin_ctz(mask)], u = rw & 0xFFFFu;
+                    const uint32_t rw = S.re[lo0 + (uint32_t)__builtin_ctz(mask)], u = rw & RM;
                     const float bx = S.pos[3 * u], by = S.pos[3 * u + 1], bz = S.pos[3 * u + 2];
                     const float sb = plane_dist(pl, bx, by, bz);
                     const float inv = 1.f / (sb - sa);
@@ -189,9 +203,9 @@
                     N.pos[3 * id] = (ax * sb - bx * sa) * inv;
                     N.pos[3 * id + 1] = (ay * sb - by * sa) * inv;
                     N.pos[3 * id + 2] = (az * sb - bz * sa) * inv;
-                    N.vw[id] = lo | (3u << 16);
-                    N.re[lo] = (nKeep + L.pred[t]) | (1u << 16); N.re[lo + 1] = (nKeep + L.succ[t]) | (0u << 16);
-                    N.re[lo + 2] = (uint32_t)L.mp[u] | (rw & 0xFFFF0000u);
+                    N.vw[id] = lo | (3u << VS);
+                    N.re[lo] = (nKeep + L.pred[t]) | (1u << RS); N.re[lo + 1] = (nKeep + L.succ[t]) | (0u << RS);
+                    N.re[lo + 2] = (uint32_t)L.mp[u] | (rw & ~RM);
                 }
             }
         }
@@ -211,25 +225,29 @@
     return 0;
 }
 
-__device__ inline SolidIn sc_stage(const ScSolid& S, uint32_t nv, float* pos, uint32_t* loff, uint32_t* llen, uint32_t* ring)
-{
+template <class SOLID>
+__device__ inline SolidIn sc_stage(const SOLID& S, uint32_t nv, float* pos, uint32_t* loff, uint32_t* llen, uint32_t* ring)
+{
+    constexpr uint32_t VS = SOLID::kVwSh, VM = (1u << VS) - 1u, RM = (1u << SOLID::kReSh) - 1u;
     for (uint32_t v = lane_id(); v < nv; v += SURTR_LANES)
     {
         pos[3 * v] = S.pos[3 * v]; pos[3 * v + 1] = S.pos[3 * v + 1]; pos[3 * v + 2] = S.pos[3 * v + 2];
-        const uint32_t w = S.vw[v], lo = w & 0xFFFFu, len = w >> 16;
+        const uint32_t w = S.vw[v], lo = w & VM, len = w >> VS;
         loff[v] = lo; llen[v] = len;
-        for (uint32_t q = 0; q < len; ++q) ring[lo + q] = S.re[lo + q] & 0xFFFFu;
+        for (uint32_t q = 0; q < len; ++q) ring[lo + q] = S.re[lo + q] & RM;
     }
     __threadfence_block();
     __syncthreads();
     return SolidIn{pos, loff, llen, (const int32_t*)ring, nv, nullptr, nullptr, nullptr, nullptr, nullptr};
 }
 
-__device__ inline int sc_park(const ScSolid& S, uint32_t nv, Shared& sh, uint32_t* cursors, float* apos, uint32_t* aloff, uint32_t* allen, int32_t* anbr,
+template <class SOLID, class SH>
+__device__ inline int sc_park(const SOLID& S, uint32_t nv, SH& sh, uint32_t* cursors, float* apos, uint32_t* aloff, uint32_t* allen, int32_t* anbr,
                               uint32_t capV, uint32_t capH, uint32_t& voff, uint32_t& n, uint32_t& hoff, uint32_t& nh)
 {
+    constexpr uint32_t VS = SOLID::kVwSh, VM = (1u << VS) - 1u, RM = (1u << SOLID::kReSh) - 1u;
     const uint32_t wl = S.vw[nv - 1u];
-    const uint32_t H = (wl & 0xFFFFu) + (wl >> 16);
+    const uint32_t H = (wl & VM) + (wl >> VS);
     __syncthreads();
     if (threadIdx.x == 0) { sh.misc[0] = atomicAdd(&cursors[CUR_V], nv); sh.misc[1] = atomicAdd(&cursors[CUR_H], H); }
     __syncthreads();
@@ -241,10 +259,10 @@
         const size_t id = (size_t)voff + v;
         apos[3 * id] = S.pos[3 * v]; apos[3 * id + 1] = S.pos[3 * v + 1]; apos[3 * id + 2] = S.pos[3 * v + 2];
         const uint32_t w = S.vw[v];
-        const uint32_t lo = hoff + (w & 0xFFFFu), len = w >> 16;
+        const uint32_t lo = hoff + (w & VM), len = w >> VS;
         aloff[id] = lo; allen[id] = len;
-        const uint32_t* r = S.re + (w & 0xFFFFu);
-        for (uint32_t q = 0; q < len; ++q) anbr[lo + q] = (int32_t)(r[q] & 0xFFFFu);
+        const typename SOLID::Word* r = S.re + (w & VM);
+        for (uint32_t q = 0; q < len; ++q) anbr[lo + q] = (int32_t)(r[q] & RM);
     }
     n = nv; nh = H;
     __syncthreads();
diff --git a/surtr_amd/csrc/surtr_ctx.h b/surtr_amd/csrc/surtr_ctx.h
--- a/surtr_amd/csrc/surtr_ctx.h
+++ b/surtr_amd/csrc/surtr_ctx.h
@@ -97,6 +97,7 @@
     CUR_BIG_QUOTA = 84,
     CUR_FACES2_N = 85,
     CUR_Q_FACES2 = 86,
+    CUR_CVX_GAVE_UP = 87,
     CUR_REC_TOOK = 88,
     CUR_REC_HANDED = 89,
     CUR_LIT_TOO_LARGE = 90,
@@ -106,6 +107,7 @@
     CUR_CATCH_CLIPPED = 94,
     CUR_UNREFITTED = 95,
     CUR_WC_WHY = 96,
+    CUR_Q_CONVEX2 = 125,
     CUR_STATS_WORDS = 128,
     CUR_HO_PUSHED = 146,
     CUR_HO_STARTED = 147,
@@ -240,7 +242,7 @@
     int device = 0;
     bool frags_of_pieces = false;
     uint32_t hw_wg = 512, hw_wg_faces = 1024, hw_wg_prep = 1792, hw_wg_big = 48, budget_vmax = 0xFFFFFFFFu, budget_hmax = 0xFFFFFFFFu;
-    uint32_t max_wg = 512, max_wg_faces = 1024, max_wg_small = 2048, max_wg_prep = 1792, max_wg_half = 1024;
+    uint32_t max_wg = 512, max_wg_faces = 1024, max_wg_small = 2048, max_wg_lean = 3072, max_wg_prep = 1792, max_wg_half = 1024;
     DevBuf<uint32_t> d_hlist;
     uint32_t vmin = 0;
     ScratchPool pool_half{}; uint32_t n_wg_half = 0; DevBuf<char> pool_half_buf;
@@ -281,6 +283,7 @@
     uint32_t regroup_rounds = 0;
     uint64_t tot_mv = 0, tot_mh = 0;
     uint32_t n_cells = 0, n_faces = 0;
+    DevBuf<uint32_t> d_cvx_giveup;
     DevBuf<uint32_t> d_pair_order; uint32_t pair_order_begin = 0, pair_order_count = 0;
     bool pair_order_is_list = false;
     DevBuf<float> d_v012; DevBuf<float4> d_planes; DevBuf<uint32_t> d_plane_off;
diff --git a/surtr_amd/csrc/surtr_hip.hip b/surtr_amd/csrc/surtr_hip.hip
--- a/surtr_amd/csrc/surtr_hip.hip
+++ b/surtr_amd/csrc/surtr_hip.hip
@@ -672,17 +672,170 @@
 #ifndef SURTR_SMALL_WAVES
 #define SURTR_SMALL_WAVES 2
 #endif
+__device__ __forceinline__ static void convex_publish(PairRec* __restrict__ pairs, uint32_t p, const PairRec& rec, uint32_t front_par)
+{
+    if (threadIdx.x != 0) return;
+    if (!front_par) pairs[p] = rec;
+    else
+    {
+        PairRec& o = pairs[p];
+        o.cv_off = rec.cv_off; o.cv_n = rec.cv_n; o.ch_off = rec.ch_off; o.ch_n = rec.ch_n;
+        o.mv_off = 0; o.mv_n = 0; o.mh_off = 0; o.mh_n = 0; o.ni = 0; o.isl_off = 0; o.status = rec.status; o.cv_bad = rec.cv_bad;
+    }
+}
+__device__ __forceinline__ static void convex_enqueue_prep(const Pieces& P, uint32_t piece, uint32_t p, uint32_t F, const float4* planes, float4* pmar,
+                                                           const Arena& A, uint32_t* __restrict__ porder, uint32_t n_pairs)
+{
+    const uint32_t tid = threadIdx.x;
+    const uint32_t m0 = P.mvo[piece], V = P.mvo[piece + 1] - m0;
+    const float4* bs = P.mbsph + P.mbo[piece];
+    const uint32_t nsb = (V + SURTR_SB - 1u) / SURTR_SB;
+    __syncthreads();
+    for (uint32_t k = tid; k < F; k += group_size())
+    {
+        const float4 pk = planes[k];
+        const float n1 = fabsf(pk.x) + fabsf(pk.y) + fabsf(pk.z);
+        const float n2 = sqrtf(pk.x * pk.x + pk.y * pk.y + pk.z * pk.z) * 1.0001f;
+        pmar[k] = make_float4(n2 * 1.00101f, 1.0e-5f * fabsf(pk.w), 1.0e-5f * n1, 0.f);
+    }
+    __syncthreads();
+    uint32_t und = 0;
+    for (uint32_t sb = tid * 8u; sb < nsb; sb += group_size() * 8u)
+    {
+        const float4 sp = bs[sb];
+        const float mag = fabsf(sp.x) + fabsf(sp.y) + fabsf(sp.z) + sp.w;
+        bool decided = false;
+        for (uint32_t k = 0; k < F; ++k)
+        {
+            const float4 mk = pmar[k];
+            const float sk = plane_dist(planes[k], sp.x, sp.y, sp.z);
+            const float margin = sp.w * mk.x + mk.y + mk.z * mag;
+            if (sk > margin) { decided = true; break; }
+            if (!(sk < -margin)) break;
+        }
+        if (!decided) ++und;
+    }
+    const uint2 tot = wave_incl_scan2(make_uint2(und, 0u));
+    if (tid == group_size() - 1u)
+    {
+        uint32_t l2 = 0; while ((tot.x >> (l2 + 1u)) != 0u) ++l2;
+        uint32_t cls = 2u * l2 + (l2 ? ((tot.x >> (l2 - 1u)) & 1u) : 0u);
+        cls = cls > 4u ? cls - 4u : 0u; if (cls > 15u) cls = 15u;
+        porder[(size_t)cls * n_pairs + atomicAdd(&A.cursors[CUR_CLS_PREP + cls], 1u)] = p;
+    }
+}
+
 __global__ __launch_bounds__(SURTR_LANES) __attribute__((amdgpu_waves_per_eu(SURTR_SMALL_WAVES, 8))) void k_clip_convex(Pieces P, const float4* __restrict__ planes,
                                                     const uint32_t* __restrict__ plane_off, uint32_t cell_begin,
                                                     uint32_t n_pairs, const uint8_t* __restrict__ outside,
                                                     ScratchPool pool, Arena A, PairRec* __restrict__ pairs,
                                                     const uint2* __restrict__ pair_list, uint32_t* __restrict__ porder,
-                                                    const uint32_t* __restrict__ pair_order, uint32_t front_par)
+                                                    const uint32_t* __restrict__ pair_order, uint32_t front_par,
+                                                    const uint32_t* __restrict__ giveup)
 {
     __shared__ Shared sh;
     __shared__ OneWaveLds U;
     LdsTopoSmall& L = U.g.L; LdsWorkSmall& W = U.g.W;
     Scratch S = carve(pool, blockIdx.x);
+    const uint32_t tid = threadIdx.x;
+    while (true)
+    {
+        __syncthreads();
+        if (tid == 0)
+        {
+            if (giveup == nullptr) sh.misc[7] = atomicAdd(&A.cursors[CUR_Q_CONVEX], 1u);
+            else
+            {
+                const uint32_t t = atomicAdd(&A.cursors[CUR_Q_CONVEX2], 1u);
+                sh.misc[7] = t < A.cursors[CUR_CVX_GAVE_UP] ? giveup[t] : 0xFFFFFFFFu;
+            }
+        }
+        __syncthreads();
+        uint32_t p = sh.misc[7];
+        if (p >= n_pairs) break;
+        if (giveup == nullptr && pair_order != nullptr) p = pair_order[p];
+        const PairAt at = pair_where(p, pair_list, cell_begin, P.n);
+        const uint32_t cell = at.cell, piece = at.piece;
+        PairRec rec;
+        memset(&rec, 0, sizeof(rec));
+#ifdef SURTR_STAMP_SMALL
+        if (tid == 0) for (int q = 0; q < 16; ++q) sh.ph[q] = 0;
+#endif
+        bool skip = outside != nullptr && outside[piece] != 0;
+        const uint32_t f0 = plane_off[cell], F = plane_off[cell + 1] - f0;
+        if (F > SURTR_MAXF) { rec.status = SURTR_E_INVALID; skip = true; }
+        int err = 0;
+        ChainStamp cst{};
+#ifdef SURTR_STAMP
+        const unsigned long long cx0 = __builtin_readcyclecounter();
+        cst.t_small = cst.t_park = cx0;
+#endif
+        if (!skip)
+        {
+            for (uint32_t k = tid; k < F; k += group_size()) sh.planes[k] = planes[f0 + k];
+            __syncthreads();
+            const ChainCaller who{CUR_CVX_TOOK, CUR_CVX_RESUMED, true, nullptr, planes + f0};
+            const ParkOut o = convex_chain(convex_solid_in(P, piece), F, P.cdup[piece] != 0, who, [&] { return LiteralArg{convex_solid_in(P, piece), false}; }, sh, U, S, pool, A, cst);
+            err = o.err; rec.cv_off = o.voff; rec.cv_n = o.n; rec.ch_off = o.hoff; rec.ch_n = o.nh;
+        }
+        if (err == SURTR_E_TOPOLOGY) { rec.cv_bad = 1; rec.cv_off = 0; rec.cv_n = 1; rec.ch_off = 0; rec.ch_n = 0; err = 0; }
+        if (err != 0) { rec.status = (uint32_t)err; rec.cv_n = 0; if (tid == 0) atomicMax(&A.cursors[CUR_STATUS], (uint32_t)err); }
+        convex_publish(pairs, p, rec, front_par);
+        if (rec.cv_n != 0 && porder != nullptr) convex_enqueue_prep(P, piece, p, F, sh.planes, sh.pmar, A, porder, n_pairs);
+#ifdef SURTR_STAMP_SMALL
+        if (tid == 0) for (int q = 0; q < 16; ++q) if (sh.ph[q]) atomicAdd(&g_stamp[q], sh.ph[q]);
+#endif
+#ifdef SURTR_STAMP
+        if (tid == 0)
+        {
+            const unsigned long long cx1 = cst.t_small, cx2 = cst.t_park, cx3 = __builtin_readcyclecounter();
+            const unsigned long long d = cx3 - cx0;
+            atomicAdd(&g_stamp2[32], d); atomicAdd(&g_stamp2[33], 1ull);
+            const unsigned long long old = atomicMax(&g_stamp2[34], d);
+            if (d > old)
+            {
+                g_stamp2[35] = cx1 - cx0; g_stamp2[36] = cx2 - cx1; g_stamp2[37] = cx3 - cx2; g_stamp2[38] = F;
+                for (int q = 0; q < 7; ++q) g_stamp2[40 + q] = U.f.tph[q];
+            }
+        }
+#endif
+    }
+}
+
+#ifndef SURTR_LEAN_WAVES
+#define SURTR_LEAN_WAVES 2
+#endif
+#ifndef SURTR_LEAN_V
+#if SURTR_LEAN_WAVES <= 2
+#define SURTR_LEAN_V SC_V
+#define SURTR_LEAN_H SC_H
+#define SURTR_LEAN_WORD uint32_t
+#elif SURTR_LEAN_WAVES == 3
+#define SURTR_LEAN_V SC_V
+#define SURTR_LEAN_H SC_H
+#define SURTR_LEAN_WORD uint16_t
+#else
+#define SURTR_LEAN_V 156u
+#define SURTR_LEAN_H 480u
+#define SURTR_LEAN_WORD uint16_t
+#endif
+#endif
+struct LeanShared { float4 planes[SURTR_MAXF + 1]; uint32_t misc[8]; };
+typedef ScLdsT<SURTR_LEAN_V, SURTR_LEAN_H, SURTR_LEAN_WORD> LeanSolidLds;
+union alignas(16) LeanLds { LeanSolidLds f; float4 pmar[SURTR_MAXF + 1]; };
+#if SURTR_LANES != 1
+static_assert((sizeof(LeanShared) + sizeof(LeanLds)) * 4u * SURTR_LEAN_WAVES <= 160u * 1024u, "LDS admits fewer workgroups per CU than the register budget");
+#endif
+__global__ __launch_bounds__(SURTR_LANES) __attribute__((amdgpu_waves_per_eu(SURTR_LEAN_WAVES, 8))) void k_clip_convex_lean(Pieces P, const float4* __restrict__ planes,
+                                                    const uint32_t* __restrict__ plane_off, uint32_t cell_begin,
+                                                    uint32_t n_pairs, const uint8_t* __restrict__ outside,
+                                                    Arena A, PairRec* __restrict__ pairs,
+                                                    const uint2* __restrict__ pair_list, uint32_t* __restrict__ porder,
+                                                    const uint32_t* __restrict__ pair_order, uint32_t front_par,
+                                                    uint32_t* __restrict__ giveup)
+{
+    __shared__ LeanShared sh;
+    __shared__ LeanLds U;
     const uint32_t tid = threadIdx.x;
     while (true)
     {
@@ -696,94 +849,36 @@
         const uint32_t cell = at.cell, piece = at.piece;
         PairRec rec;
         memset(&rec, 0, sizeof(rec));
-#ifdef SURTR_STAMP_SMALL
-        if (tid == 0) for (int q = 0; q < 16; ++q) sh.ph[q] = 0;
-#endif
         bool skip = outside != nullptr && outside[piece] != 0;
         const uint32_t f0 = plane_off[cell], F = plane_off[cell + 1] - f0;
         if (F > SURTR_MAXF) { rec.status = SURTR_E_INVALID; skip = true; }
-        int err = 0;
-        ChainStamp cst{};
-#ifdef SURTR_STAMP
-        const unsigned long long cx0 = __builtin_readcyclecounter();
-        cst.t_small = cst.t_park = cx0;
-#endif
         if (!skip)
         {
-            for (uint32_t k = tid; k < F; k += group_size()) sh.planes[k] = planes[f0 + k];
-            __syncthreads();
-            const ChainCaller who{CUR_CVX_TOOK, CUR_CVX_RESUMED, true, nullptr, planes + f0};
-            const ParkOut o = convex_chain(convex_solid_in(P, piece), F, P.cdup[piece] != 0, who, [&] { return LiteralArg{convex_solid_in(P, piece), false}; }, sh, U, S, pool, A, cst);
-            err = o.err; rec.cv_off = o.voff; rec.cv_n = o.n; rec.ch_off = o.hoff; rec.ch_n = o.nh;
-        }
-        if (err == SURTR_E_TOPOLOGY) { rec.cv_bad = 1; rec.cv_off = 0; rec.cv_n = 1; rec.ch_off = 0; rec.ch_n = 0; err = 0; }
-        if (err != 0) { rec.status = (uint32_t)err; rec.cv_n = 0; if (tid == 0) atomicMax(&A.cursors[CUR_STATUS], (uint32_t)err); }
-        if (tid == 0)
-        {
-            if (!front_par) pairs[p] = rec;
-            else
-            {
-                PairRec& o = pairs[p];
-                o.cv_off = rec.cv_off; o.cv_n = rec.cv_n; o.ch_off = rec.ch_off; o.ch_n = rec.ch_n;
-                o.mv_off = 0; o.mv_n = 0; o.mh_off = 0; o.mh_n = 0; o.ni = 0; o.isl_off = 0; o.status = rec.status; o.cv_bad = rec.cv_bad;
-            }
-        }
-        if (rec.cv_n != 0 && porder != nullptr)
-        {
-            const uint32_t m0 = P.mvo[piece], V = P.mvo[piece + 1] - m0;
-            const float4* bs = P.mbsph + P.mbo[piece];
-            const uint32_t nsb = (V + SURTR_SB - 1u) / SURTR_SB;
-            __syncthreads();
-            for (uint32_t k = tid; k < F; k += group_size())
-            {
-                const float4 pk = sh.planes[k];
-                const float n1 = fabsf(pk.x) + fabsf(pk.y) + fabsf(pk.z);
-                const float n2 = sqrtf(pk.x * pk.x + pk.y * pk.y + pk.z * pk.z) * 1.0001f;
-                sh.pmar[k] = make_float4(n2 * 1.00101f, 1.0e-5f * fabsf(pk.w), 1.0e-5f * n1, 0.f);
-            }
-            __syncthreads();
-            uint32_t und = 0;
-            for (uint32_t sb = tid * 8u; sb < nsb; sb += group_size() * 8u)
-            {
-                const float4 sp = bs[sb];
-                const float mag = fabsf(sp.x) + fabsf(sp.y) + fabsf(sp.z) + sp.w;
-                bool decided = false;
-                for (uint32_t k = 0; k < F; ++k)
+            int err = SC_FALLBACK;
+            uint32_t voff = 0, n = 0, hoff = 0, nh = 0;
+            if (P.cdup[piece] == 0)
+            {
+                for (uint32_t k = tid; k < F; k += group_size()) sh.planes[k] = planes[f0 + k];
+                __syncthreads();
+                uint32_t which = 0;
+                err = small_clip(convex_solid_in(P, piece), F, sh, U.f, &which);
+                if (err == 0)
                 {
-                    const float4 mk = sh.pmar[k];
-                    const float sk = plane_dist(sh.planes[k], sp.x, sp.y, sp.z);
-                    const float margin = sp.w * mk.x + mk.y + mk.z * mag;
-                    if (sk > margin) { decided = true; break; }
-                    if (!(sk < -margin)) break;
+                    const uint32_t nv = U.f.nv[which];
+                    if (nv != 0u) err = sc_park(U.f.buf[which], nv, sh, A.cursors, A.pos, A.loff, A.llen, A.nbr, A.capV, A.capH, voff, n, hoff, nh);
                 }
-                if (!decided) ++und;
-            }
-            const uint2 tot = wave_incl_scan2(make_uint2(und, 0u));
-            if (tid == group_size() - 1u)
-            {
-                uint32_t l2 = 0; while ((tot.x >> (l2 + 1u)) != 0u) ++l2;
-                uint32_t cls = 2u * l2 + (l2 ? ((tot.x >> (l2 - 1u)) & 1u) : 0u);
-                cls = cls > 4u ? cls - 4u : 0u; if (cls > 15u) cls = 15u;
-                porder[(size_t)cls * n_pairs + atomicAdd(&A.cursors[CUR_CLS_PREP + cls], 1u)] = p;
-            }
-        }
-#ifdef SURTR_STAMP_SMALL
-        if (tid == 0) for (int q = 0; q < 16; ++q) if (sh.ph[q]) atomicAdd(&g_stamp[q], sh.ph[q]);
-#endif
-#ifdef SURTR_STAMP
-        if (tid == 0)
-        {
-            const unsigned long long cx1 = cst.t_small, cx2 = cst.t_park, cx3 = __builtin_readcyclecounter();
-            const unsigned long long d = cx3 - cx0;
-            atomicAdd(&g_stamp2[32], d); atomicAdd(&g_stamp2[33], 1ull);
-            const unsigned long long old = atomicMax(&g_stamp2[34], d);
-            if (d > old)
-            {
-                g_stamp2[35] = cx1 - cx0; g_stamp2[36] = cx2 - cx1; g_stamp2[37] = cx3 - cx2; g_stamp2[38] = F;
-                for (int q = 0; q < 7; ++q) g_stamp2[40 + q] = U.f.tph[q];
-            }
-        }
-#endif
+                __syncthreads();
+            }
+            if (err != 0)
+            {
+                if (tid == 0) giveup[atomicAdd(&A.cursors[CUR_CVX_GAVE_UP], 1u)] = p;
+                continue;
+            }
+            if (tid == 0) atomicAdd(&A.cursors[CUR_CVX_TOOK], 1u);
+            rec.cv_off = voff; rec.cv_n = n; rec.ch_off = hoff; rec.ch_n = nh;
+        }
+        convex_publish(pairs, p, rec, front_par);
+        if (rec.cv_n != 0 && porder != nullptr) convex_enqueue_prep(P, piece, p, F, sh.planes, U.pmar, A, porder, n_pairs);
     }
 }
 
@@ -2864,6 +2959,7 @@
             uint32_t small_per_cu = 8u;
             if (const char* e = getenv("SURTR_SMALL_PER_CU")) { const int v = atoi(e); if (v > 0 && v <= 32) small_per_cu = (uint32_t)v; }
             ctx->max_wg_small = (uint32_t)prop.multiProcessorCount * small_per_cu;
+            ctx->max_wg_lean = (uint32_t)prop.multiProcessorCount * 4u * SURTR_LEAN_WAVES;
             uint32_t prep_per_cu = SURTR_PREP_WAVES;
             if (const char* e = getenv("SURTR_PREP_PER_CU")) { const int v = atoi(e); if (v > 0 && v <= 32) prep_per_cu = (uint32_t)v; }
             ctx->max_wg_prep = (uint32_t)prop.multiProcessorCount * prep_per_cu;
@@ -3177,7 +3273,8 @@
         ctx->arena = Arena{B.pos, B.loff, B.llen, B.nbr, B.idx, B.isl, (uint32_t)av, (uint32_t)ah, (uint32_t)ai, capIsl, B.cursors};
         ctx->cap_frags = capIsl;
     }
-    const int rc = ctx->d_pairs.grow(ctx, n_pairs);
+    int rc = ctx->d_pairs.grow(ctx, n_pairs);
+    if (rc == SURTR_OK) rc = ctx->d_cvx_giveup.grow(ctx, n_pairs);
     if (rc) return rc;
     return ctx->d_scanblk.grow(ctx, std::max(n_pairs, ctx->cap_frags) / SURTR_LANES + 4);
 }
@@ -3214,9 +3311,10 @@
     decltype(&k_prep_pairs) prep;
     uint32_t prep_threads;
     bool wave_on, split_on, use_half, front_par, both;
+    bool cvx_lean;
     uint32_t rec_on;
     uint32_t big_quota, big_n, walk0, n_catch, n_poll;
-    uint32_t n_wg, n_wg_cvx, n_wg_prep, n_wg_big, n_wg_half, n_wg_retry, n_wg_sweep;
+    uint32_t n_wg, n_wg_cvx, n_wg_lean, n_wg_cvx2, n_wg_prep, n_wg_big, n_wg_half, n_wg_retry, n_wg_sweep;
     uint32_t g_refit, g_faces, t_faces;
     hipStream_t st_cvx, st_main, st_bigk, st_refit;
 };
@@ -3228,6 +3326,8 @@
     pl.cell_order = !pair_list && n_pairs && ctx->n_pieces && n_pairs % ctx->n_pieces == 0 && !getenv("SURTR_NO_CELL_ORDER");
     pl.n_wg = std::max(1u, std::min(n1, max_wg));
     pl.n_wg_cvx = std::max(1u, std::min(n1, ctx->max_wg_small));
+    pl.n_wg_lean = std::max(1u, std::min(n1, ctx->max_wg_lean));
+    pl.n_wg_cvx2 = std::min(n1, 64u);
     pl.n_wg_half = std::max(1u, std::min(n1, ctx->max_wg_half));
     pl.n_wg_prep = std::max(1u, std::min(n1, ctx->max_wg_prep));
     pl.n_wg_big = std::min(ctx->n_wg_big, n1);
@@ -3259,6 +3359,8 @@
     pl.front_par = n_pairs != 0 && n_pairs <= SURTR_FRONT_PAR_MAX && !prep_wide;
     if (const char* e = getenv("SURTR_FRONT_PAR")) pl.front_par = n_pairs != 0 && atoi(e) != 0;
     if (pl.front_par) pl.rec_on |= 4u;
+    pl.cvx_lean = n_pairs > ctx->max_wg_small;
+    if (const char* e = getenv("SURTR_CVX_LEAN")) pl.cvx_lean = n_pairs != 0 && atoi(e) != 0;
     pl.prep = nullptr; pl.prep_threads = SURTR_WG;
     if (n_pairs && prep_wide) { pl.prep = k_prep_pairs_wide; pl.prep_threads = SURTR_WG_WIDE; }
     else if (n_pairs && !(pl.rec_on & 2u) && ctx->vmax < 0xFFFFu && ctx->vmin >= SURTR_PREP_MINV && (ctx->vmax + SURTR_LANES - 1u) / SURTR_LANES <= SURTR_PREP_NB)
@@ -3373,10 +3475,19 @@
         HIPCHK(hipStreamWaitEvent(pl.st_cvx, ctx->ev_prep, 0));
     }
     PROF_BEGIN_ON(6, pl.st_cvx);
-    if (n_pairs)
+    if (n_pairs && pl.cvx_lean)
+    {
+        uint32_t* const cvx_porder = pl.front_par ? (uint32_t*)nullptr : porder;
+        hipLaunchKernelGGL(k_clip_convex_lean, dim3(pl.n_wg_lean), dim3(SURTR_LANES), 0, pl.st_cvx, P, ctx->d_planes, ctx->d_plane_off, cell_begin, n_pairs,
+                           d_out, ctx->arena, ctx->d_pairs, d_pair_list, cvx_porder, d_pair_order, pl.front_par ? 1u : 0u, (uint32_t*)ctx->d_cvx_giveup);
+        hipLaunchKernelGGL(k_clip_convex, dim3(pl.n_wg_cvx2), dim3(SURTR_LANES), 0, pl.st_cvx, P, ctx->d_planes, ctx->d_plane_off, cell_begin, n_pairs,
+                           d_out, ctx->pool_small, ctx->arena, ctx->d_pairs, d_pair_list, cvx_porder, (const uint32_t*)nullptr,
+                           pl.front_par ? 1u : 0u, (const uint32_t*)ctx->d_cvx_giveup);
+    }
+    else if (n_pairs)
         hipLaunchKernelGGL(k_clip_convex, dim3(pl.n_wg_cvx), dim3(SURTR_LANES), 0, pl.st_cvx, P, ctx->d_planes, ctx->d_plane_off, cell_begin, n_pairs,
                            d_out, ctx->pool_small, ctx->arena, ctx->d_pairs, d_pair_list, pl.front_par ? (uint32_t*)nullptr : porder, d_pair_order,
-                           pl.front_par ? 1u : 0u);
+                           pl.front_par ? 1u : 0u, (const uint32_t*)nullptr);
     PROF_END_ON(6, pl.st_cvx);
     if (pl.front_par) HIPCHK(hipEventRecord(ctx->ev_cvx, pl.st_cvx));
     PROF_BEGIN(7);
```

Result: faster. 1.196 million, median of 6 (+5.5%).
